# facebookresearch/wmar

Hardware: AMD Instinct MI355X
Metric: watermarked images/sec at 256x256 (16x16 tok), batch 64; detector p-value delta vs ref (higher is better)
Workload: dtype f32; 1 GPU; Taming cin_transformer (48L x 1536d x 24h, V=16384) + VQGAN f16/16384, 256x256, batch 64 per GPU, greenlist watermark delta=2 gamma=0.25 h=1 (linear/stratifiedrand), T=1 top-k 250 top-p 0.92; sample -> decode -> re-encode -> detect; random-init weights; batch_per_gpu=64, decode_loop=hipGraph replay, backend=nccl

## Files before the change

### include/wmar_hip.h

```cpp
#ifndef WMAR_HIP_H
#define WMAR_HIP_H

#include <stdint.h>

#ifdef __cplusplus
extern "C" {
#endif

#define WMAR_OK 0
#define WMAR_EINVAL (-1)
#define WMAR_EHIP (-2)
#define WMAR_ESHORT (-3)
#define WMAR_MAX_CONTEXT 16
#define WMAR_ENOMEM (-4)
#define WMAR_EMISSING (-5)
#define WMAR_ECALLBACK (-6)

#define WMAR_SEED_FIXED 0
#define WMAR_SEED_LINEAR 1
#define WMAR_SEED_SPATIAL 2
#define WMAR_SPLIT_RAND 0
#define WMAR_SPLIT_STRATIFIED 1

const char* wmar_last_error(void);
int wmar_version(void);

typedef struct wmar_key_params {
    uint64_t salt_key;
    const int64_t* alive_ids;
    int64_t n_alive;
    const int64_t* dead_ids;
    int64_t n_dead;
    int64_t vocab_size;
    double gamma;
    int32_t split_strategy;
    int32_t seed_strategy;
} wmar_key_params;

int64_t wmar_key_row_words(int64_t vocab_size);
int64_t wmar_key_table_rows(int32_t seed_strategy, int32_t context_size, int64_t max_token);
int wmar_key_table_build(const wmar_key_params* key, int64_t row0, int64_t n_rows, uint32_t* out_host,
                         int32_t n_threads);
int64_t wmar_key_greenlist(const wmar_key_params* key, uint64_t seed, int64_t* out_ids_host);

typedef struct wmar_wm_ctx {
    const uint32_t* table_dev;
    int64_t n_rows;
    int64_t vocab_size;
    int32_t seed_strategy;
    int32_t context_size;
    int32_t spatial_dim;
    float delta;
} wmar_wm_ctx;

int wmar_wm_process_logits(const wmar_wm_ctx* wm, float* logits_dev, int64_t B, const int64_t* past_ids_dev,
                           int64_t t, int64_t past_stride, void* stream);

int wmar_sample_fused(const wmar_wm_ctx* wm, const float* logits_dev, int64_t B, int64_t V,
                      const int64_t* past_ids_dev, int64_t t, int64_t past_stride, float temperature,
                      int32_t top_k, double top_p, const float* q_dev, float* scratch_dev,
                      int64_t* tok_out_dev, void* stream);

int wmar_detect(const wmar_wm_ctx* wm, double gamma, const int64_t* codes_dev, int64_t B, int64_t L,
                int32_t* n_scored_dev, int32_t* n_green_dev, double* pval_dev, int8_t* mask_dev,
                int64_t mask_stride, void* stream);
int64_t wmar_detect_num_ngrams(int32_t seed_strategy, int32_t context_size, int64_t L);

typedef struct wmar_gpt_config {
    int32_t vocab_size, block_size, n_layer, n_head, n_embd;
    int32_t max_batch;
} wmar_gpt_config;

typedef struct wmar_gpt wmar_gpt;

int wmar_gpt_create(const wmar_gpt_config* cfg, const char* const* names, const void* const* tensors_dev,
                    int32_t n_tensors, void* stream, wmar_gpt** out);
void wmar_gpt_destroy(wmar_gpt* g);
int64_t wmar_gpt_device_bytes(const wmar_gpt* g);

int wmar_gpt_decode_step(wmar_gpt* g, const int64_t* tok_dev, int64_t B, int32_t pos, float* logits_dev,
                         void* stream);

typedef struct wmar_sample_params {
    float temperature;
    int32_t top_k;
    double top_p;
    int32_t use_graph;
} wmar_sample_params;

int wmar_gpt_generate(wmar_gpt* g, const wmar_wm_ctx* wm, const wmar_sample_params* sp, const int64_t* cond_dev,
                      int64_t B, int32_t steps, const float* q_dev, int64_t* tokens_out_dev,
                      float* logits_trace_dev, void* stream);

typedef int (*wmar_logits_hook)(void* user, int32_t step, int64_t t);

int wmar_cfg_mix(const float* cond_dev, const float* img_dev, const float* uncond_dev, float* out_dev, int64_t B, int64_t V,
                 const float* scale_dev, const int32_t* step_dev, float g_text, float g_image, void* stream);

int wmar_gpt_generate_hooked(wmar_gpt* g, const wmar_sample_params* sp, const int64_t* cond_dev, int64_t B, int32_t steps,
                             const float* q_dev, int64_t* tokens_out_dev, float* logits_io_dev, int64_t* past_io_dev,
                             int64_t past_stride, wmar_logits_hook hook, void* user, void* stream);

#define WMAR_T_EMBED 0
#define WMAR_T_QKV 1
#define WMAR_T_ATTN 2
#define WMAR_T_PROJ 3
#define WMAR_T_RESID 4
#define WMAR_T_FC1 5
#define WMAR_T_FC2 6
#define WMAR_T_HEAD 7
#define WMAR_T_SAMPLE 8
#define WMAR_T_NCLASS 9
int wmar_gpt_check(wmar_gpt* g, void* stream);
int wmar_gpt_set_timing(wmar_gpt* g, int32_t enabled);
int wmar_gpt_set_attention_phases(wmar_gpt* g, int32_t one_wave_upto, int32_t two_waves_upto);
int wmar_gpt_profile_role(wmar_gpt* g, int32_t role, int64_t B, int32_t kv_len, int32_t iters, void* stream,
                          double* avg_us);
int wmar_gpt_plan_info(wmar_gpt* g, int64_t B, char* buf, int64_t buf_len);
int wmar_gpt_get_timing(wmar_gpt* g, double* total_us, int64_t* calls, double* step_ms);

typedef struct wmar_rar_config {
    int32_t hidden_size, num_hidden_layers, num_attention_heads, intermediate_size;
    int32_t image_seq_len, codebook_size, condition_num_classes;
    int32_t max_batch;
} wmar_rar_config;

typedef struct wmar_rar wmar_rar;

int wmar_rar_create(const wmar_rar_config* cfg, const char* const* names, const void* const* tensors_dev,
                    int32_t n_tensors, void* stream, wmar_rar** out);
void wmar_rar_destroy(wmar_rar* g);
int64_t wmar_rar_device_bytes(const wmar_rar* g);

int wmar_rar_forward_position(wmar_rar* g, const int64_t* tok_dev, const int64_t* cond_ids_dev, int64_t M, int32_t pos,
                              float* logits_dev, void* stream);

int wmar_rar_generate(wmar_rar* g, const wmar_wm_ctx* wm, const int64_t* class_ids_dev, int64_t B,
                      const float* cfg_scale_host, int32_t use_guidance, float temperature, const float* q_dev,
                      int64_t* tokens_out_dev, int32_t use_graph, void* stream);

int wmar_rar_generate_hooked(wmar_rar* g, const int64_t* class_ids_dev, int64_t B, const float* cfg_scale_host,
                             int32_t use_guidance, float temperature, const float* q_dev, int64_t* tokens_out_dev,
                             int32_t use_graph, float* logits_io_dev, int64_t* past_io_dev, int64_t past_stride,
                             wmar_logits_hook hook, void* user, void* stream);

// ... 159 lines not shown
```

### wmar_amd/_lib.py

```python
from __future__ import annotations

import ctypes as C
import os

HERE = os.path.dirname(os.path.abspath(__file__))
LIB_PATH = os.path.join(HERE, "libwmar_hip.so")

SYMBOLS = [
    "wmar_last_error", "wmar_version", "wmar_key_row_words", "wmar_key_table_rows", "wmar_key_table_build",
    "wmar_key_greenlist", "wmar_wm_process_logits", "wmar_sample_fused", "wmar_detect", "wmar_detect_num_ngrams",
    "wmar_gpt_create", "wmar_gpt_destroy", "wmar_gpt_device_bytes", "wmar_gpt_decode_step", "wmar_gpt_generate",
    "wmar_gpt_set_timing", "wmar_gpt_set_attention_phases", "wmar_gpt_get_timing", "wmar_gpt_profile_role", "wmar_gpt_plan_info", "wmar_gpt_check", "wmar_rar_create", "wmar_rar_destroy",
    "wmar_rar_device_bytes", "wmar_rar_forward_position", "wmar_rar_generate", "wmar_vq_create", "wmar_vq_destroy", "wmar_vq_device_bytes",
    "wmar_vq_decode", "wmar_vq_encode", "wmar_vq_probe_conv", "wmar_vq_probe_attn", "wmar_vq_probe_argmin", "wmar_mvq_create", "wmar_mvq_destroy", "wmar_mvq_device_bytes", "wmar_mvq_decode",
    "wmar_mvq_encode", "wmar_gumbel_key_build", "wmar_gumbel_sample", "wmar_gumbel_score", "wmar_gumbel_key_rows", "wmar_gumbel_score_ctx", "wmar_rar_generate_gumbel", "wmar_rar_generate_gumbel_ctx", "wmar_rar_check", "wmar_rar_launch_status",
    "wmar_cham_create", "wmar_cham_destroy", "wmar_cham_device_bytes", "wmar_cham_forward_tokens", "wmar_cham_generate_image",
    "wmar_cham_sample",
    "wmar_cfg_mix", "wmar_gpt_generate_hooked", "wmar_rar_generate_hooked", "wmar_cham_generate_image_hooked",
    "wmar_augment", "wmar_jpeg_workspace_bytes", "wmar_jpeg", "wmar_resample_coeffs", "wmar_image_ingest",
    "wmar_sync_positions", "wmar_sync_workspace_bytes", "wmar_sync_fit", "wmar_sync_rotate_labels",
    "wmar_comm_unique_id", "wmar_comm_init", "wmar_comm_bcast", "wmar_comm_allgather", "wmar_comm_rank", "wmar_comm_world", "wmar_comm_destroy",
]

WMAR_ESHORT = -3
WMAR_ECALLBACK = -6

LOGITS_HOOK = C.CFUNCTYPE(C.c_int, C.c_void_p, C.c_int32, C.c_int64)


class KeyParams(C.Structure):
    _fields_ = [("salt_key", C.c_uint64), ("alive_ids", C.POINTER(C.c_int64)), ("n_alive", C.c_int64),
                ("dead_ids", C.POINTER(C.c_int64)), ("n_dead", C.c_int64), ("vocab_size", C.c_int64),
                ("gamma", C.c_double), ("split_strategy", C.c_int32), ("seed_strategy", C.c_int32)]


class WmCtx(C.Structure):
    _fields_ = [("table_dev", C.c_void_p), ("n_rows", C.c_int64), ("vocab_size", C.c_int64),
                ("seed_strategy", C.c_int32), ("context_size", C.c_int32), ("spatial_dim", C.c_int32),
                ("delta", C.c_float)]


class GptConfig(C.Structure):
    _fields_ = [("vocab_size", C.c_int32), ("block_size", C.c_int32), ("n_layer", C.c_int32),
                ("n_head", C.c_int32), ("n_embd", C.c_int32), ("max_batch", C.c_int32)]


class RarConfig(C.Structure):
    _fields_ = [("hidden_size", C.c_int32), ("num_hidden_layers", C.c_int32), ("num_attention_heads", C.c_int32),
                ("intermediate_size", C.c_int32), ("image_seq_len", C.c_int32), ("codebook_size", C.c_int32),
                ("condition_num_classes", C.c_int32), ("max_batch", C.c_int32)]


class SampleParams(C.Structure):
    _fields_ = [("temperature", C.c_float), ("top_k", C.c_int32), ("top_p", C.c_double), ("use_graph", C.c_int32)]


class VqConfig(C.Structure):
    _fields_ = [("ch", C.c_int32), ("num_res_blocks", C.c_int32), ("resolution", C.c_int32),
                ("in_channels", C.c_int32), ("out_ch", C.c_int32), ("z_channels", C.c_int32),
                ("embed_dim", C.c_int32), ("n_embed", C.c_int32), ("n_levels", C.c_int32),
                ("ch_mult", C.c_int32 * 8), ("n_attn_res", C.c_int32), ("attn_resolutions", C.c_int32 * 8),
                ("max_batch", C.c_int32)]


class MvqConfig(C.Structure):
    _fields_ = [("hidden_channels", C.c_int32), ("num_res_blocks", C.c_int32), ("resolution", C.c_int32),
                ("num_channels", C.c_int32), ("z_channels", C.c_int32), ("num_embeddings", C.c_int32),
                ("n_levels", C.c_int32), ("channel_mult", C.c_int32 * 8), ("max_batch", C.c_int32)]


class ChamConfig(C.Structure):
    _fields_ = [("dim", C.c_int32), ("n_layers", C.c_int32), ("n_heads", C.c_int32), ("n_kv_heads", C.c_int32),
                ("vocab_size", C.c_int32), ("ffn_hidden", C.c_int32), ("norm_eps", C.c_float), ("rope_theta", C.c_float),
                ("qk_normalization", C.c_int32), ("swin_norm", C.c_int32), ("max_rows", C.c_int32),
                ("max_seq_len", C.c_int32), ("tensors_bf16", C.c_int32)]


class ChamSampleParams(C.Structure):
    _fields_ = [("temperature", C.c_float), ("top_p", C.c_double), ("guidance_scale_text", C.c_float),
                ("guidance_scale_image", C.c_float), ("use_graph", C.c_int32), ("pad_id", C.c_int32)]


class ImageDesc(C.Structure):
    _fields_ = [("offset", C.c_int64), ("width", C.c_int32), ("height", C.c_int32), ("channels", C.c_int32),
                ("new_width", C.c_int32), ("new_height", C.c_int32), ("crop_x0", C.c_int32), ("crop_y0", C.c_int32)]


class WmarError(RuntimeError):
    def __init__(self, code, msg):
        super().__init__(f"libwmar_hip: {msg} (status {code})")
        self.code = code


_LIB = None


def load():
    global _LIB
    if _LIB is not None:
        return _LIB
    import torch

    if not os.path.exists(LIB_PATH):
        raise ImportError(
            f"{LIB_PATH} is missing: build it with `python -m wmar_amd.build` (hipcc, gfx950). "
            "wmar_amd has no CPU fallback.")
    L = C.CDLL(LIB_PATH, mode=C.RTLD_GLOBAL)
    vp, i64, i32, f32, f64 = C.c_void_p, C.c_int64, C.c_int32, C.c_float, C.c_double
    L.wmar_last_error.restype = C.c_char_p
    L.wmar_key_row_words.restype = i64
    L.wmar_key_row_words.argtypes = [i64]
    L.wmar_key_table_rows.restype = i64
    L.wmar_key_table_rows.argtypes = [i32, i32, i64]
    L.wmar_key_table_build.argtypes = [C.POINTER(KeyParams), i64, i64, vp, i32]
    L.wmar_key_greenlist.restype = i64
    L.wmar_key_greenlist.argtypes = [C.POINTER(KeyParams), C.c_uint64, vp]
    L.wmar_wm_process_logits.argtypes = [C.POINTER(WmCtx), vp, i64, vp, i64, i64, vp]
    L.wmar_sample_fused.argtypes = [C.POINTER(WmCtx), vp, i64, i64, vp, i64, i64, f32, i32, f64, vp, vp, vp, vp]
    L.wmar_detect.argtypes = [C.POINTER(WmCtx), f64, vp, i64, i64, vp, vp, vp, vp, i64, vp]
    L.wmar_detect_num_ngrams.restype = i64
    L.wmar_detect_num_ngrams.argtypes = [i32, i32, i64]
    L.wmar_augment.argtypes = [i32, vp, vp, vp, i64, i32, i32, i32, i32, f64, f64, vp]
    L.wmar_jpeg_workspace_bytes.restype = i64
    L.wmar_jpeg_workspace_bytes.argtypes = [i64, i32, i32]
    L.wmar_jpeg.argtypes = [vp, vp, vp, i64, i64, i32, i32, i32, i32, i32, vp]
    L.wmar_resample_coeffs.argtypes = [i32, i32, i32, i32, vp, vp, vp, i32, C.POINTER(i32)]
    L.wmar_image_ingest.argtypes = [vp, i64, C.POINTER(ImageDesc), i64, i32, vp, vp, vp]
    L.wmar_sync_positions.argtypes = [vp, i64, i32, vp, vp, vp]
    L.wmar_sync_workspace_bytes.restype = i64
    L.wmar_sync_workspace_bytes.argtypes = [i64, i32]
    L.wmar_sync_fit.argtypes = [vp, i64, i32, vp, vp, vp, i64, vp]
    L.wmar_sync_rotate_labels.argtypes = [vp, i64, i32, i32, vp, vp, i64, vp]
    L.wmar_comm_unique_id.argtypes = [vp, i64]
    L.wmar_comm_init.argtypes = [vp, i64, i32, i32, C.POINTER(vp)]
    L.wmar_comm_bcast.argtypes = [vp, vp, i64, i32, vp]
    L.wmar_comm_allgather.argtypes = [vp, vp, vp, i64, vp]
    L.wmar_comm_rank.argtypes = [vp]
    L.wmar_comm_rank.restype = i32
    L.wmar_comm_world.argtypes = [vp]
    L.wmar_comm_world.restype = i32
    L.wmar_comm_destroy.argtypes = [vp]
    L.wmar_comm_destroy.restype = None
    L.wmar_gpt_create.argtypes = [C.POINTER(GptConfig), C.POINTER(C.c_char_p), C.POINTER(vp), i32, vp, C.POINTER(vp)]
    L.wmar_gpt_destroy.argtypes = [vp]
    L.wmar_gpt_destroy.restype = None
    L.wmar_gpt_device_bytes.restype = i64
    L.wmar_gpt_device_bytes.argtypes = [vp]
    L.wmar_gpt_decode_step.argtypes = [vp, vp, i64, i32, vp, vp]
    L.wmar_gpt_generate.argtypes = [vp, C.POINTER(WmCtx), C.POINTER(SampleParams), vp, i64, i32, vp, vp, vp, vp]
    L.wmar_gpt_set_timing.argtypes = [vp, i32]
    L.wmar_gpt_set_attention_phases.argtypes = [vp, i32, i32]
    L.wmar_gpt_profile_role.argtypes = [vp, i32, i64, i32, i32, vp, C.POINTER(f64)]
    L.wmar_gpt_get_timing.argtypes = [vp, C.POINTER(f64), C.POINTER(i64), C.POINTER(f64)]
    L.wmar_gpt_plan_info.argtypes = [vp, i64, C.c_char_p, i64]
    L.wmar_gpt_check.argtypes = [vp, vp]
    L.wmar_rar_create.argtypes = [C.POINTER(RarConfig), C.POINTER(C.c_char_p), C.POINTER(vp), i32, vp, C.POINTER(vp)]
    L.wmar_rar_destroy.argtypes = [vp]
    L.wmar_rar_destroy.restype = None
    L.wmar_rar_device_bytes.restype = i64
    L.wmar_rar_device_bytes.argtypes = [vp]
    L.wmar_rar_forward_position.argtypes = [vp, vp, vp, i64, i32, vp, vp]
    L.wmar_rar_generate.argtypes = [vp, C.POINTER(WmCtx), vp, i64, C.POINTER(f32), i32, f32, vp, vp, i32, vp]
    L.wmar_rar_generate_gumbel.argtypes = [vp, vp, i64, C.POINTER(f32), i32, f32, f32, i32, vp, vp, i32, vp]
    L.wmar_rar_generate_gumbel_ctx.argtypes = [vp, vp, i64, C.POINTER(f32), i32, f32, f32, i32, C.c_uint64, i32, vp, vp, i32, vp]
    L.wmar_rar_check.argtypes = [vp, vp]
    L.wmar_rar_launch_status.argtypes = [vp, C.POINTER(i32), C.POINTER(i32)]
    L.wmar_gumbel_key_build.argtypes = [C.c_uint64, i64, vp, vp, vp]
    L.wmar_gumbel_sample.argtypes = [vp, i64, i64, vp, i64, i32, f32, f32, i32, vp, vp]
    L.wmar_gumbel_score.argtypes = [vp, i64, i64, i64, vp, i64, vp, vp, vp]
    L.wmar_gumbel_key_rows.argtypes = [vp, i64, i64, vp, vp, vp, vp]
    L.wmar_gumbel_score_ctx.argtypes = [vp, i64, i64, i64, C.c_uint64, i32, vp, vp, vp, vp]
    if hasattr(L, "wmar_vq_create"):
        L.wmar_vq_create.argtypes = [C.POINTER(VqConfig), C.POINTER(C.c_char_p), C.POINTER(vp), i32, vp, C.POINTER(vp)]
        L.wmar_vq_destroy.argtypes = [vp]
        L.wmar_vq_destroy.restype = None
        L.wmar_vq_device_bytes.restype = i64
        L.wmar_vq_device_bytes.argtypes = [vp]
        L.wmar_vq_decode.argtypes = [vp, vp, i64, vp, vp]
        L.wmar_vq_encode.argtypes = [vp, vp, i64, vp, vp, vp]
        L.wmar_vq_probe_conv.argtypes = [vp, vp, i32, i32, i32, vp, vp, vp, vp, i32, i64, i32, i32, i32, i32, i32, vp, vp, C.c_char_p, i64, vp]
        L.wmar_vq_probe_attn.argtypes = [vp, vp, vp, i64, i32, i32, i32, vp, C.c_char_p, i64, vp]
        L.wmar_vq_probe_argmin.argtypes = [vp, i64, i32, vp, i32, vp, C.c_char_p, i64, vp]
    L.wmar_cham_create.argtypes = [C.POINTER(ChamConfig), C.POINTER(C.c_char_p), C.POINTER(vp), i32, vp, C.POINTER(vp)]
    L.wmar_cham_destroy.argtypes = [vp]
    L.wmar_cham_destroy.restype = None
    L.wmar_cham_device_bytes.restype = i64
    L.wmar_cham_device_bytes.argtypes = [vp]
    L.wmar_cham_forward_tokens.argtypes = [vp, vp, vp, i64, vp, vp]
    L.wmar_cham_generate_image.argtypes = [vp, C.POINTER(WmCtx), vp, vp, i64, C.POINTER(ChamSampleParams), vp, vp, i32, vp, i32, vp, vp]
    L.wmar_cham_sample.argtypes = [C.POINTER(WmCtx), vp, i64, i64, vp, i64, i64, f32, f64, f32, f32, vp, vp, i32, vp, vp, vp, vp]
    L.wmar_cfg_mix.argtypes = [vp, vp, vp, vp, i64, i64, vp, vp, f32, f32, vp]
    L.wmar_gpt_generate_hooked.argtypes = [vp, C.POINTER(SampleParams), vp, i64, i32, vp, vp, vp, vp, i64, LOGITS_HOOK, vp, vp]
    L.wmar_rar_generate_hooked.argtypes = [vp, vp, i64, C.POINTER(f32), i32, f32, vp, vp, i32, vp, vp, i64, LOGITS_HOOK, vp, vp]
    L.wmar_cham_generate_image_hooked.argtypes = [vp, vp, vp, i64, C.POINTER(ChamSampleParams), vp, vp, i32, vp, i32, vp, vp, vp, i64,
                                                  LOGITS_HOOK, vp, vp]
    L.wmar_mvq_create.argtypes = [C.POINTER(MvqConfig), C.POINTER(C.c_char_p), C.POINTER(vp), i32, vp, C.POINTER(vp)]
    L.wmar_mvq_destroy.argtypes = [vp]
    L.wmar_mvq_destroy.restype = None
    L.wmar_mvq_device_bytes.restype = i64
    L.wmar_mvq_device_bytes.argtypes = [vp]
    L.wmar_mvq_decode.argtypes = [vp, vp, i64, vp, vp]
    L.wmar_mvq_encode.argtypes = [vp, vp, i64, vp, vp, vp]
    _LIB = L
# ... 23 lines not shown
```

### wmar_amd/csrc/decoder_kernels.h

```cpp
#pragma once
#include <cstdint>

#include "sampler.h"
#include "bx_split.h"

namespace wmar {

using f32x16 = __attribute__((ext_vector_type(16))) float;
using f32x4 = __attribute__((ext_vector_type(4))) float;

__device__ __forceinline__ float4 ld_nt(const float4* p) {
    f32x4 v = __builtin_nontemporal_load((const f32x4*)p);
    return make_float4(v.x, v.y, v.z, v.w);
}

__device__ __forceinline__ void st_out(float4* p, const float4 v) {
#ifndef WMAR_PLAIN_STORES
    const f32x4 q = {v.x, v.y, v.z, v.w};
    asm volatile("global_store_dwordx4 %0, %1, off sc1\n\ts_nop 1" :: "v"(p), "v"(q) : "memory");
#else
    *p = v;
#endif
}
using f32x2 = __attribute__((ext_vector_type(2))) float;
// ... 649 lines not shown
        mu = (float)mean;
        rstd = rsqrtf((float)var_f64(sq * invK, mean) + 1e-5f);
    }
    for (int gi = w; gi < 6; gi += 4) {
        float o[4] = {0.f, 0.f, 0.f, 0.f};
#pragma unroll
        for (int ww = 0; ww < 4; ++ww) {
            const float4 t = red[ww][gi][lane];
            o[0] += t.x; o[1] += t.y; o[2] += t.z; o[3] += t.w;
        }
        const int m = gi < 4 ? 16 * gi + (lane & 15) : lane;
        const int n = tile * 24 + (gi < 4 ? 4 * (lane >> 4) : 16 + 4 * (gi - 4));
        const float mm = __shfl(mu, m), rs = __shfl(rstd, m);
        const float4 cc = gi < 4 ? ccA_ : ccB_;
        const float4 bb = gi < 4 ? bbA_ : bbB_;
        o[0] = gelu_erf(rs * (o[0] - mm * cc.x) + bb.x); o[1] = gelu_erf(rs * (o[1] - mm * cc.y) + bb.y);
        o[2] = gelu_erf(rs * (o[2] - mm * cc.z) + bb.z); o[3] = gelu_erf(rs * (o[3] - mm * cc.w) + bb.w);
        st_out(a.out + ((long long)(n >> 3) * 2 + (m >> 5)) * 64 + (m & 31) + 32 * ((n >> 2) & 1), make_float4(o[0], o[1], o[2], o[3]));
    }
    WMAR_ST_END(a.trace, blockIdx.x)
#ifdef WMAR_FX_TRACE
    if (a.trace && threadIdx.x == 0) {
        asm volatile("s_waitcnt vmcnt(0)" ::: "memory");
        unsigned long long* t = a.trace + (long long)blockIdx.x * 4;
        t[0] = tr0; t[1] = tr1; t[2] = tr2; t[3] = __builtin_amdgcn_s_memtime();
    }
#endif
}

constexpr int QX_CK = 4;
#ifndef QX_ABL
#define QX_ABL 0
#endif
#define WMAR_QX_SYNC() if (!(QX_ABL & 2)) __syncthreads();
#ifndef QX_SPLIT
#define QX_SPLIT 2
#endif

struct QkvxArgs {
    const float4* Wp;
    const float4* x_in;
    float4* x_out;
    const float4* slabs;
    long long slab_stride;
    int n_hi;
    const float* bias;
    double* stats;
    float4* out;
    long long out_stride;
    int KB, NT, S, cap;
    int nkeep;
    unsigned long long* trace;
    unsigned long long* trace_chunks;
};

template <int MTW, int S_IN>
__global__ __launch_bounds__(512) void k_qkvx(QkvxArgs a) {
    __shared__ __attribute__((aligned(16))) float4 xs[2][QX_CK][MTW][64];
    __shared__ double red[4][MTW][64][2];
    const int lane = threadIdx.x & 63;
    const int w = __builtin_amdgcn_readfirstlane(threadIdx.x >> 6);
    const int half = lane >> 5;
    const int G = a.NT >> 2;
    const int j = (int)(blockIdx.x & 7) * a.cap + (int)(blockIdx.x >> 3);
    if (j >= G * a.S) return;
    const int s = j / G, g = j - s * G;
    const int kb0 = (int)((unsigned)s * (unsigned)a.KB / (unsigned)a.S);
    const int kb1 = (int)((unsigned)(s + 1) * (unsigned)a.KB / (unsigned)a.S);
    const int nkb = kb1 - kb0, nch = (nkb + QX_CK - 1) / QX_CK;
    const bool keeper = g == 0;

    if (w >= 4) {
        const int sw = w - 4;
        double sum[MTW], sq[MTW];
#pragma unroll
        for (int i = 0; i < MTW; ++i) { sum[i] = 0.0; sq[i] = 0.0; }
        float4 xvA[MTW], bbA, slA[S_IN > 0 ? S_IN : 1][MTW];
        float4 xvB[MTW], bbB, slB[S_IN > 0 ? S_IN : 1][MTW];
        int skbA = 0, skbB = 0;
#define WMAR_QX_ISSUE(XV, BB, SL, SKB, C)                                                              \
    {                                                                                                   \
        SKB = kb0 + (C) * QX_CK + sw;                                                                   \
        const int kk = SKB < kb1 ? SKB : kb1 - 1;                                                       \
        const long long idx = (long long)kk * MTW * 64 + lane;                                          \
        _Pragma("unroll") for (int i = 0; i < MTW; ++i) XV[i] = a.x_in[idx + i * 64];                   \
        if (S_IN > 0) {                                                                                 \
            BB = *(const float4*)(a.bias + kk * 8 + 4 * half);                                          \
            _Pragma("unroll") for (int si = 0; si < S_IN; ++si)                                         \
                _Pragma("unroll") for (int i = 0; i < MTW; ++i)                                         \
                    SL[si][i] = a.slabs[(long long)si * a.slab_stride + idx + i * 64];                  \
        }                                                                                               \
    }
#define WMAR_QX_FINISH(XV, BB, SL, SKB, BUF)                                                           \
    if (SKB < kb1) {                                                                                    \
        const bool short_tile = a.n_hi > 0 && (SKB >> 2) >= a.n_hi;                                     \
        _Pragma("unroll") for (int i = 0; i < MTW; ++i) {                                               \
            float4 r = XV[i];                                                                           \
            if (S_IN > 0) {                                                                             \
                float4 t = SL[0][i];                                                                    \
                _Pragma("unroll") for (int si = 1; si < S_IN; ++si)                                     \
                    if (!(si == S_IN - 1 && short_tile)) {                                              \
                        t.x += SL[si][i].x; t.y += SL[si][i].y; t.z += SL[si][i].z; t.w += SL[si][i].w; \
                    }                                                                                   \
                r = make_float4(r.x + (BB.x + t.x), r.y + (BB.y + t.y), r.z + (BB.z + t.z), r.w + (BB.w + t.w)); \
            }                                                                                           \
            xs[BUF][sw][i][lane] = r;                                                                   \
// ... 129 lines not shown
#endif
#pragma unroll
    for (int i = 0; i < MTW; ++i)
#pragma unroll
        for (int q4 = 0; q4 < 4; ++q4)
            st_out(a.out + (long long)s * a.out_stride + ((long long)(nt * 4 + q4) * MTW + i) * 64 + lane,
                   make_float4(acc[i][q4 * 4 + 0], acc[i][q4 * 4 + 1], acc[i][q4 * 4 + 2], acc[i][q4 * 4 + 3]));
    if (keeper) __syncthreads();
#ifdef WMAR_QX_TRACE
    if (a.trace && lane == 0) {
        asm volatile("s_waitcnt vmcnt(0)" ::: "memory");
        unsigned long long* t = a.trace + ((long long)j * 4 + w) * 4;
        t[0] = tr0; t[1] = tr1; t[2] = tr2; t[3] = __builtin_amdgcn_s_memtime();
        if (a.trace_chunks) for (int i = 0; i < 8; ++i) a.trace_chunks[((long long)j * 4 + w) * 8 + i] = trc[i] ? trc[i] - tr1 : 0;
    }
#endif
}

template <int MTW>
static int launch_qkvx_mt(const QkvxArgs& q, int S_in, hipStream_t st) {
    const dim3 grid((unsigned)(8 * q.cap));
    switch (S_in) {
#define WMAR_QX_CASE(N) case N: hipLaunchKernelGGL((k_qkvx<MTW, N>), grid, dim3(512), 0, st, q); break;
        WMAR_QX_CASE(0) WMAR_QX_CASE(1) WMAR_QX_CASE(2) WMAR_QX_CASE(3) WMAR_QX_CASE(4)
        WMAR_QX_CASE(5) WMAR_QX_CASE(6) WMAR_QX_CASE(7) WMAR_QX_CASE(8)
#undef WMAR_QX_CASE
        default: set_error("qkvx: bad slab count %d", S_in); return WMAR_EINVAL;
    }
    return launch_status("k_qkvx");
}
static int launch_qkvx(const QkvxArgs& q, int MT, int S_in, hipStream_t st) {
    if (MT == 1) return launch_qkvx_mt<1>(q, S_in, st);
    if (MT == 2) return launch_qkvx_mt<2>(q, S_in, st);
    set_error("qkvx: %d row tiles unsupported", MT);
    return WMAR_EINVAL;
}

static __global__ void k_pack_bx(const float* __restrict__ W, const float* __restrict__ gamma, float4* __restrict__ Wq, int N, int K,
                                      int tile_off) {
    const long long idx = (long long)blockIdx.x * blockDim.x + threadIdx.x;
    const int KU = K / 16;
    if (idx >= (long long)(N / 32) * KU * 128) return;
    const int lane = (int)(idx & 63), hf = (int)((idx >> 6) & 1);
    const long long r = idx >> 7;
    const int ku = (int)(r % KU), tile = (int)(r / KU);
    const int k = ku * 16 + 8 * (lane >> 5) + 4 * hf;
    const float* p = W + (long long)(tile * 32 + (lane & 31)) * K + k;
    float4 v = make_float4(p[0], p[1], p[2], p[3]);
    if (gamma) { v.x *= gamma[k]; v.y *= gamma[k + 1]; v.z *= gamma[k + 2]; v.w *= gamma[k + 3]; }
    Wq[idx + (long long)tile_off * KU * 128] = v;
}

constexpr int QX_TR_STRIDE = 36;
template <int S_IN>
__global__ __launch_bounds__(512) void k_qkvx_bx(QkvxArgs a) {
    constexpr int MTW = 2;
    __shared__ __attribute__((aligned(16))) u32x4 xq[2][2][MTW][3][64];
    __shared__ __attribute__((aligned(16))) float tr_s[4][32 * QX_TR_STRIDE];
    __shared__ double red[4][MTW][64][2];
    const int lane = threadIdx.x & 63;
    const int w = __builtin_amdgcn_readfirstlane(threadIdx.x >> 6);
    const int half = lane >> 5;
    const int G = a.NT >> 2;
    const int j = (int)(blockIdx.x & 7) * a.cap + (int)(blockIdx.x >> 3);
    if (j >= G * a.S) return;
    const int s = j / G, g = j - s * G;
    const int KU = a.KB >> 1;
    const int kb0 = 2 * (int)((unsigned)s * (unsigned)KU / (unsigned)a.S);
    const int kb1 = 2 * (int)((unsigned)(s + 1) * (unsigned)KU / (unsigned)a.S);
    const int nkb = kb1 - kb0, nch = (nkb + QX_CK - 1) / QX_CK;
    const bool keeper = g < a.nkeep;

    if (w >= 4) {
        const int sw = w - 4;
        double sum[MTW], sq[MTW];
#pragma unroll
        for (int i = 0; i < MTW; ++i) { sum[i] = 0.0; sq[i] = 0.0; }
        float4 xvA[MTW], bbA, slA[S_IN > 0 ? S_IN : 1][MTW];
        float4 xvB[MTW], bbB, slB[S_IN > 0 ? S_IN : 1][MTW];
        int skbA = 0, skbB = 0;
#define WMAR_QX_ISSUE(XV, BB, SL, SKB, C)                                                              \
    {                                                                                                   \
        SKB = kb0 + (C) * QX_CK + sw;                                                                   \
        const int kk = SKB < kb1 ? SKB : kb1 - 1;                                                       \
        const long long idx = (long long)kk * MTW * 64 + lane;                                          \
        _Pragma("unroll") for (int i = 0; i < MTW; ++i) XV[i] = a.x_in[idx + i * 64];                   \
        if (S_IN > 0) {                                                                                 \
            BB = *(const float4*)(a.bias + kk * 8 + 4 * half);                                          \
            _Pragma("unroll") for (int si = 0; si < S_IN; ++si)                                         \
                _Pragma("unroll") for (int i = 0; i < MTW; ++i)                                         \
                    SL[si][i] = a.slabs[(long long)si * a.slab_stride + idx + i * 64];                  \
        }                                                                                               \
    }
#define WMAR_QX_FINISH(XV, BB, SL, SKB, BUF, CIDX)                                                     \
    if (SKB < kb1) {                                                                                    \
        const bool short_tile = a.n_hi > 0 && (SKB >> 2) >= a.n_hi;                                     \
        _Pragma("unroll") for (int i = 0; i < MTW; ++i) {                                               \
            float4 r = XV[i];                                                                           \
            if (S_IN > 0) {                                                                             \
                float4 t = SL[0][i];                                                                    \
                _Pragma("unroll") for (int si = 1; si < S_IN; ++si)                                     \
                    if (!(si == S_IN - 1 && short_tile)) {                                              \
                        t.x += SL[si][i].x; t.y += SL[si][i].y; t.z += SL[si][i].z; t.w += SL[si][i].w; \
                    }                                                                                   \
                r = make_float4(r.x + (BB.x + t.x), r.y + (BB.y + t.y), r.z + (BB.z + t.z), r.w + (BB.w + t.w)); \
            }                                                                                           \
            unsigned h0, m0, l0, h1, m1, l1;                                                            \
            bx_split2(r.x, r.y, h0, m0, l0);                                                            \
            bx_split2(r.z, r.w, h1, m1, l1);                                                            \
            u32x2* d = (u32x2*)&xq[BUF][sw >> 1][i][0][(lane & 31) + 32 * (sw & 1)] + half;             \
            d[0] = u32x2{h0, h1}; d[128] = u32x2{m0, m1}; d[256] = u32x2{l0, l1};                       \
            if (keeper && (CIDX) % a.nkeep == g) {                                                      \
                a.x_out[((long long)SKB * MTW + i) * 64 + lane] = r;                                    \
                sum[i] += (double)r.x + (double)r.y + (double)r.z + (double)r.w;                        \
                sq[i] += sq4_f64(r);                        \
            }                                                                                           \
        }                                                                                               \
    }
        WMAR_QX_ISSUE(xvA, bbA, slA, skbA, 0)
        WMAR_QX_ISSUE(xvB, bbB, slB, skbB, 1)
        __builtin_amdgcn_sched_barrier(0);
        WMAR_QX_FINISH(xvA, bbA, slA, skbA, 0, 0)
        __builtin_amdgcn_sched_barrier(0);
        WMAR_QX_ISSUE(xvA, bbA, slA, skbA, 2)
        __builtin_amdgcn_sched_barrier(0);
        __syncthreads();
        for (int c = 0; c + 1 < nch; c += 2) {
            WMAR_QX_FINISH(xvB, bbB, slB, skbB, 1, c + 1)
            __builtin_amdgcn_sched_barrier(0);
            WMAR_QX_ISSUE(xvB, bbB, slB, skbB, c + 3)
            __builtin_amdgcn_sched_barrier(0);
            __syncthreads();
            if (c + 2 >= nch) break;
            WMAR_QX_FINISH(xvA, bbA, slA, skbA, 0, c + 2)
            __builtin_amdgcn_sched_barrier(0);
            WMAR_QX_ISSUE(xvA, bbA, slA, skbA, c + 4)
            __builtin_amdgcn_sched_barrier(0);
            __syncthreads();
        }
#undef WMAR_QX_ISSUE
#undef WMAR_QX_FINISH
        if (keeper) {
#pragma unroll
            for (int i = 0; i < MTW; ++i) {
                red[sw][i][lane][0] = sum[i]; red[sw][i][lane][1] = sq[i];
            }
            __syncthreads();
            const int t = threadIdx.x - 256;
            if (t < 32 * MTW) {
                const int i = t >> 5, r = t & 31;
                double ts = 0, tss = 0;
// ... 49 lines not shown
    __builtin_amdgcn_sched_barrier(0);                                                                  \
    if ((C) + 1 < nch) {                                                                                \
        __syncthreads();                                                                                \
        WMAR_QX_READ(XNEXT, BUFNEXT)                                                                    \
    }                                                                                                   \
    __builtin_amdgcn_sched_barrier(0);                                                                  \
    WMAR_QX_MMA(WCUR, XCUR, C, 1)                                                                       \
    __builtin_amdgcn_sched_barrier(0);

    WMAR_QX_W(w0, 0)
    WMAR_QX_W(w1, 1)
    WMAR_QX_W(w2, 2)
    __syncthreads();
    WMAR_ST_LANDED(2)
    WMAR_QX_READ(xfA, 0)
    for (int c = 0; c < nch; c += 4) {
        WMAR_QX_STEP(c, w0, w3, xfA, xfB, 1)
        if (c + 1 >= nch) break;
        WMAR_QX_STEP(c + 1, w1, w0, xfB, xfA, 0)
        if (c + 2 >= nch) break;
        WMAR_QX_STEP(c + 2, w2, w1, xfA, xfB, 1)
        if (c + 3 >= nch) break;
        WMAR_QX_STEP(c + 3, w3, w2, xfB, xfA, 0)
    }
    WMAR_ST(3)
#undef WMAR_QX_W
#undef WMAR_QX_READ
#undef WMAR_QX_MMA
#undef WMAR_QX_MFMA
#undef WMAR_QX_BF
#undef WMAR_QX_STEP
#pragma unroll
    for (int i = 0; i < MTW; ++i) {
        float* T = &tr_s[w][0];
#pragma unroll
        for (int q4 = 0; q4 < 4; ++q4)
            *(float4*)(T + (lane & 31) * QX_TR_STRIDE + 8 * q4 + 4 * half) =
                make_float4(acc[i][q4 * 4 + 0], acc[i][q4 * 4 + 1], acc[i][q4 * 4 + 2], acc[i][q4 * 4 + 3]);
        __builtin_amdgcn_wave_barrier();
        asm volatile("s_waitcnt lgkmcnt(0)" ::: "memory");
#pragma unroll
        for (int it = 0; it < 4; ++it) {
            const int row = (lane >> 3) + 8 * it, cg = lane & 7;
            const float4 v = *(const float4*)(T + row * QX_TR_STRIDE + 4 * cg);
            st_out(a.out + (long long)s * a.out_stride + ((long long)(32 * i + row) * (a.NT * 32) + nt * 32 + 4 * cg) / 4, v);
        }
        __builtin_amdgcn_wave_barrier();
        asm volatile("s_waitcnt lgkmcnt(0)" ::: "memory");
    }
    WMAR_ST_END(a.trace, j)
    if (keeper) __syncthreads();
}

static int launch_qkvx_bx(const QkvxArgs& q, int S_in, hipStream_t st) {
    const dim3 grid((unsigned)(8 * q.cap));
    switch (S_in) {
#define WMAR_QX_CASE(N) case N: hipLaunchKernelGGL((k_qkvx_bx<N>), grid, dim3(512), 0, st, q); break;
        WMAR_QX_CASE(0) WMAR_QX_CASE(1) WMAR_QX_CASE(2) WMAR_QX_CASE(3) WMAR_QX_CASE(4)
        WMAR_QX_CASE(5) WMAR_QX_CASE(6) WMAR_QX_CASE(7) WMAR_QX_CASE(8)
#undef WMAR_QX_CASE
        default: set_error("qkvx_bx: bad slab count %d", S_in); return WMAR_EINVAL;
    }
    return launch_status("k_qkvx_bx");
}


struct BxArgs {
    const float4* Wq;
    const u32x4* Xq;
    float4* out;
    long long slab_stride;
    int KU;
    int S;
    const float* bias;
    u32x4* outq;
    int rowmajor;
    int N;
};

#define WMAR_BX_MFMA(A, B, C) C = __builtin_amdgcn_mfma_f32_32x32x16_bf16(A, B, C, 0, 0, 0)

template <int NT, int PER, int MTW = 2, bool GELU = false, int NW = 4, bool XF = false>
__global__ __launch_bounds__(NW * 64) void k_bx(BxArgs a) {
    constexpr int XR = XF ? 2 * MTW : 3 * MTW;
    constexpr int ROWS = NT * 4 * MTW;
    __shared__ __attribute__((aligned(16))) float4 red[NW][ROWS][64];
    const int lane = threadIdx.x & 63;
    const int w = __builtin_amdgcn_readfirstlane(threadIdx.x >> 6);
    const int grp = (int)blockIdx.x / a.S, ks = (int)blockIdx.x % a.S;
    const int u0 = (ks * NW + w) * PER;
    f32x16 acc[NT][MTW];
#pragma unroll
    for (int t = 0; t < NT; ++t)
#pragma unroll
        for (int i = 0; i < MTW; ++i)
#pragma unroll
            for (int r = 0; r < 16; ++r) acc[t][i][r] = 0.f;
    const float4* wp = a.Wq + ((long long)grp * NT * a.KU + u0) * 128 + lane;
    const long long wt = (long long)a.KU * 128;
    const u32x4* xp = XF ? a.Xq + ((long long)(2 * u0 + (lane >> 5)) * MTW) * 64 + (lane & 31)
                         : a.Xq + (long long)u0 * XR * 64 + lane;
    float4 wr[NT][2];
    u32x4 xr[XR], xr2[XF ? XR : 1];
#define WMAR_BX_LOADW(U)                                                                           \
    { _Pragma("unroll") for (int t = 0; t < NT; ++t) {                                             \
        wr[t][0] = ld_nt(wp + t * wt + (long long)(U) * 128);                                      \
        wr[t][1] = ld_nt(wp + t * wt + (long long)(U) * 128 + 64); } }
#define WMAR_BX_LOADXF(XB, U)                                                                      \
// ... 809 lines not shown
```

### wmar_amd/csrc/gpt.hip

```cpp
#include <cstdint>
#include <map>
#include <string>
#include <vector>

#include "decoder_host.h"
#include "decode_small.h"
#include "decode_persist.h"


using namespace wmar;

struct LayerW {
    float4 *wqkv, *wproj, *wfc1, *wfc2;
    float4* wfc1x16 = nullptr;
    float2* wfc1x8 = nullptr;
    float4* wqkvx_bx = nullptr;
    float4* wproj_bx = nullptr;
    float *bqkv, *bproj, *bfc1, *bfc2, *cqkv, *cfc1;
};

struct SmallW {
    float *wqkv = nullptr, *bqkv = nullptr, *wproj = nullptr, *bproj = nullptr, *wfc1 = nullptr, *bfc1 = nullptr, *wfc2 = nullptr, *bfc2 = nullptr;
    float *ln1w = nullptr, *ln1b = nullptr, *ln2w = nullptr, *ln2b = nullptr;
};

struct wmar_gpt {
    wmar_gpt_config cfg{};
    int D = 0, H = 0, hd = 0, V = 0, L = 0, Tmax = 0, Bmax = 0, MTmax = 0;
    DeviceArena mem;
    std::vector<LayerW> layers;
    std::vector<SmallW> sw;
    float *whead_rm = nullptr, *lnfw = nullptr, *lnfb = nullptr;
    float *xs = nullptr, *ys = nullptr, *hs = nullptr, *qs = nullptr;
    bool small_ok = false;
    float* sw_arena = nullptr;
    unsigned* ss_bar = nullptr;
    bool persist_ok = false;
    bool ps_enqueued = false;
    bool xr_enqueued = false;
    float *tok_emb = nullptr, *pos_emb = nullptr, *bhead = nullptr, *chead = nullptr;
    float4* whead = nullptr;
    float4 *x = nullptr, *x2 = nullptr, *y = nullptr, *hbuf = nullptr, *slabs = nullptr, *qkv_slabs = nullptr;
    u32x4* yq = nullptr;
    float* qbuf = nullptr;
    double* stats = nullptr;
    double* stats_q = nullptr;
    float *kcache = nullptr, *vcache = nullptr;
    float *logits = nullptr, *scratch = nullptr;
    long long* past = nullptr;
    int *pos_dev = nullptr, *step_dev = nullptr;
    hipEvent_t ev0 = nullptr;
    static constexpr int N_PHASE = 3;
    GraphSlots<N_PHASE> gr;
    GraphSlots<N_PHASE + 1> grh;
    unsigned long long hook_key[12] = {0};
    int att_nw = 2;
    unsigned long long graph_key[12] = {0};
    int att_t1 = 1 << 30, att_t2 = 1 << 30;
    bool att_user = false;
    int att_phase(int kv, int64_t B) const {
        if (!att_user && B * H < 512) return kv <= 128 ? 1 : 2;
        return kv <= att_t1 ? 0 : (kv <= att_t2 ? 1 : 2);
    }
    static int phase_waves(int ph) { return ph == 0 ? 1 : (ph == 1 ? 2 : 4); }
    int timing = 0;
    bool no_bx_qkv = false, no_bx_proj = false;
    unsigned* xsync = nullptr;
    bool xcd_ok = false;
    bool no_xr = false;
    int inject_fail = 0;
    int fallbacks = 0;
    unsigned long long* dbg_sums = nullptr; int dbg_slot = 0;
    unsigned long long* stamps = nullptr;
    unsigned long long* stamp_slot(int l, int role) const {
        return stamps ? stamps + ((long long)(l * 5 + role) * WMAR_STAMP_UNITS) * 8 : nullptr;
    }
    bool no_bx = false;
    int force_s[3] = {0, 0, 0};
    double step_ms = 0.0;
    struct Span { int cls; hipEvent_t a, b; };
    std::vector<Span> spans;
    std::vector<hipEvent_t> ev_pool;
    size_t ev_used = 0;
    bool span_on = false;
    double cls_us[WMAR_T_NCLASS] = {0};
    int64_t cls_calls[WMAR_T_NCLASS] = {0};
    hipEvent_t next_event() {
        if (ev_used == ev_pool.size()) {
            hipEvent_t e = nullptr;
            (void)hipEventCreate(&e);
            ev_pool.push_back(e);
        }
        return ev_pool[ev_used++];
    }
    void span_begin(int cls, hipStream_t st) {
        if (!span_on) return;
        Span s{cls, next_event(), next_event()};
        (void)hipEventRecord(s.a, st);
        spans.push_back(s);
    }
    void span_end(hipStream_t st) {
// ... 45 lines not shown
    ResidArgs r{};
    int S_qkv = 1, S_proj = 1, S_fc2 = 1;
    int fc2_hi = 0;
    int S_qx = 0;
    float4* xcur = nullptr;
    bool proj_bx = false;
    bool proj_xr = false;
    int nch_ln2 = 0;
    bool small = false;
    bool persist = false;

    StepPlan(wmar_gpt* g_, int64_t B_, const StepIO& io_, hipStream_t st_) : g(g_), B(B_), io(io_), st(st_) {
        small = B <= SG_MAX_ROWS && g->small_ok;
        persist = small && B <= SS_MAX_ROWS && g->persist_ok;
        MT = mt_for(B); D = g->D; KBD = D / 8; KBF = 4 * D / 8; nch = stat_chunks(KBD);
        act = (long long)KBD * MT * 64;
        r.x = g->x; r.stats = g->stats; r.KB = KBD; r.MT = MT; r.n_chunks = nch;
        r.tok_emb = g->tok_emb; r.pos_emb = g->pos_emb; r.tok = io.tok; r.tok_stride = io.tok_stride;
        r.tok_use_pos = io.tok_use_pos; r.pos_dev = g->pos_dev; r.B = (int)B; r.K = D;
        r.slabs = g->slabs; r.slab_stride = act;
        xcur = g->x;
        S_qkv = g->force_s[0] > 0 ? (g->force_s[0] > QKV_SLABS_MAX ? QKV_SLABS_MAX : g->force_s[0]) : 1;
        S_proj = g->force_s[1] > 0 ? g->force_s[1] : split_for(D / 32, KBD);
        S_fc2 = g->force_s[2] > 0 ? g->force_s[2] : ((MT % 2 == 0 && KBF >= 128) ? 4 : split_for(D / 32, KBF));
        if (g->force_s[2] <= 0 && MT == 2 && KBF >= 256) {
            const int NTd = D / 32;
            const int Slo = 256 / NTd;
            if (Slo >= 2 && Slo < MAX_SLABS && NTd * Slo <= 256) { S_fc2 = Slo; fc2_hi = 256 - NTd * Slo; if (fc2_hi >= NTd) fc2_hi = 0; }
        }
        const int NTq = 3 * D / 32;
        if (g->force_s[0] <= 0 && NTq % 4 == 0 && MT <= 2 && S_fc2 + (fc2_hi > 0 ? 1 : 0) <= MAX_SLABS) {
            const int G = NTq / 4;
            int S = 256 / G;
            if (S > QKV_SLABS_MAX) S = QKV_SLABS_MAX;
            if (S > KBD / QX_CK) S = KBD / QX_CK;
            if (S >= 1) S_qx = S;
        }
        proj_bx = MT == 2 && g->yq && g->layers[0].wproj_bx && !g->no_bx && !g->no_bx_proj && g->force_s[1] <= 0;
        if (proj_bx) S_proj = D / BX_KSLICE;
        proj_xr = proj_bx && g->xcd_ok && !g->no_xr && S_proj == 4 && (D / 32) % 8 == 0 && (D / 32 / 8) * S_proj <= 32 && (D / 32 / 8) % 2 == 0;
        nch_ln2 = proj_xr ? 16 : nch;
    }
    void dbg(const void* p, long long bytes) {
#ifdef WMAR_DEV_KNOBS
        if (!g->dbg_sums || g->dbg_slot >= 4096) return;
        hipLaunchKernelGGL(k_dbg_sum, dim3(512), dim3(256), 0, st, (const uint32_t*)p, bytes / 4, g->dbg_sums + g->dbg_slot++);
#else
        (void)p; (void)bytes;
#endif
    }
    bool qkv_bx() const { return S_qx > 0 && MT == 2 && g->layers[0].wqkvx_bx && !g->no_bx && !g->no_bx_qkv; }
    bool fc1_x() const { return MT == 2 && g->layers[0].wfc1x16 && nch_ln2 <= 16; }
    int qx_nkeep() const { const int G = 3 * D / 128; return G >= 4 && S_qx * 4 <= STAT_CHUNKS_MAX ? 4 : 1; }
    static bool head_narrow() { static int v = -1; if (v < 0) v = getenv("WMAR_HEAD_NARROW") ? 1 : 0; return v != 0; }
    int split_for(int NT, int KB) const { return pick_split(MT % 2 == 0 ? NT * (MT / 2) : NT * MT, KB, 4); }
    GemmArgs base() const {
        GemmArgs a{};
        a.MT = MT; a.B = (int)B; a.stats = g->stats; a.n_chunks = nch; a.K = D;
        a.pos_dev = g->pos_dev; a.D = D; a.H = g->H; a.hd = g->hd; a.Tmax = g->Tmax;
        return a;
    }
    SgArgs sg_base() const {
        SgArgs a{};
        a.pos_dev = g->pos_dev; a.D = D; a.H = g->H; a.Tmax = g->Tmax;
        return a;
    }
    int embed() {
        if (small) {
            SeArgs e{g->tok_emb, g->pos_emb, g->xs, io.tok, io.tok_stride, io.tok_use_pos, g->pos_dev, D};
            g->span_begin(WMAR_T_EMBED, st);
            hipLaunchKernelGGL(k_sembed, dim3((unsigned)((D / 4 + 255) / 256), (unsigned)B), dim3(256), 0, st, e);
            g->span_end(st);
            return launch_status("k_sembed");
        }
        r.x = xcur;
        g->span_begin(WMAR_T_EMBED, st);
        hipLaunchKernelGGL((k_resid_stats<true, 0>), dim3(nch * MT), dim3(256), 0, st, r);
        g->span_end(st);
        return launch_status("k_resid_stats<embed>");
    }
    int resid(const float* bias, int S, int n_hi = 0) {
        r.x = xcur;
        r.S = S + (n_hi > 0 ? 1 : 0); r.bias = bias; r.n_hi = n_hi;
        g->span_begin(WMAR_T_RESID, st);
        int rc = launch_resid(r, nch * MT, st);
        g->span_end(st);
        return rc;
    }
    int qkvx(int l, const float* prev_bias) {
        QkvxArgs q{};
        const LayerW& w = g->layers[l];
        float4* xout = (xcur == g->x) ? g->x2 : g->x;
        q.Wp = w.wqkv; q.x_in = xcur; q.x_out = xout;
        q.slabs = g->slabs; q.slab_stride = act;
        const int S_in = prev_bias ? S_fc2 + (fc2_hi > 0 ? 1 : 0) : 0;
        q.n_hi = prev_bias ? fc2_hi : 0; q.bias = prev_bias;
        q.stats = g->stats_q; q.out = g->qkv_slabs; q.out_stride = 3 * act;
        q.KB = KBD; q.NT = 3 * D / 32; q.S = S_qx;
        q.cap = ((q.NT / 4) * q.S + 7) / 8;
        q.nkeep = qx_nkeep();
        q.trace = g->stamp_slot(l, 0);
        g->span_begin(WMAR_T_QKV, st);
        int rc;
        if (qkv_bx()) { q.Wp = w.wqkvx_bx; rc = launch_qkvx_bx(q, S_in, st); }
        else rc = launch_qkvx(q, MT, S_in, st);
        g->span_end(st);
        xcur = xout;
        return rc;
    }
    int qkv_small(int l) {
        const SmallW& w = g->sw[l];
        const long long lstride = (long long)g->Bmax * g->H * g->Tmax * g->hd;
        SgArgs a = sg_base();
        a.W = w.wqkv; a.bias = g->layers[l].bqkv; a.c1 = g->layers[l].cqkv; a.x = g->xs; a.gamma = w.ln1w; a.out = g->qs;
        a.kcache = g->kcache + l * lstride; a.vcache = g->vcache + l * lstride; a.N = 3 * D; a.K = D;
        g->span_begin(WMAR_T_QKV, st);
        const int rc = launch_sgemv<3, 3, SG_QKV>(a, (int)B, st);
        g->span_end(st);
        return rc;
    }
    int qkv(int l) {
        GemmArgs a = base();
        const LayerW& w = g->layers[l];
        a.Wp = w.wqkv; a.Xp = xcur; a.KB = KBD; a.NT = 3 * D / 32;
        a.out_packed = g->qkv_slabs; a.slab_stride = 3 * act;
        int S = 1;
        g->span_begin(WMAR_T_QKV, st);
        int rc = gemm_split(a, &S, st, S_qkv);
        g->span_end(st);
        return rc;
    }
    int attn(int l) {
        const LayerW& w = g->layers[l];
        const long long lstride = (long long)g->Bmax * g->H * g->Tmax * g->hd;
        if (small) {
            SaArgs s{g->qs, g->kcache + l * lstride, g->vcache + l * lstride, g->ys, g->pos_dev, g->H, g->Tmax, D, 1.0f / sqrtf((float)g->hd)};
            g->span_begin(WMAR_T_ATTN, st);
            hipLaunchKernelGGL(k_sattn, dim3((unsigned)(B * g->H)), dim3(256), 0, st, s);
            g->span_end(st);
            return launch_status("k_sattn");
        }
        AttnArgs t{};
        t.qkv_slabs = g->qkv_slabs; t.slab_stride = 3 * act; t.K = D; t.invK = 1.0 / (double)D;
        if (S_qx > 0) { t.S = S_qx; t.stats = g->stats_q; t.n_chunks = qkv_bx() ? S_qx * qx_nkeep() : S_qx; }
        else { t.S = S_qkv; t.stats = g->stats; t.n_chunks = nch; }
        t.c1 = w.cqkv; t.bias = w.bqkv;
        t.rowmajor = qkv_bx() ? 1 : 0;
        t.kcache = g->kcache + l * lstride; t.vcache = g->vcache + l * lstride; t.y = g->y; t.yq = proj_bx ? g->yq : nullptr; t.pos_dev = g->pos_dev;
        t.D = D; t.H = g->H; t.Tmax = g->Tmax; t.MT = MT; t.scale = 1.0f / sqrtf((float)g->hd);
        t.trace = g->stamp_slot(l, 1);
        int nwa = g->att_nw;
#ifdef WMAR_DEV_KNOBS
        { const char* e = getenv("WMAR_ATT_DBG"); t.dbg = e ? atoi(e) : 0; }
        { const char* e = getenv("WMAR_ATT_NW"); if (e) nwa = atoi(e); }
#endif
        const dim3 grid((unsigned)(B * g->H));
        g->span_begin(WMAR_T_ATTN, st);
// ... 111 lines not shown
            a.W = g->whead_rm; a.bias = g->bhead; a.c1 = g->chead; a.x = g->xs; a.gamma = g->lnfw; a.out = io.logits; a.N = g->V; a.K = D;
            g->span_begin(WMAR_T_HEAD, st);
            const int rc = launch_sgemv<4, 8, SG_HEAD>(a, (int)B, st);
            g->span_end(st);
            return rc;
        }
        GemmArgs h = base();
        h.Wp = g->whead; h.Xp = xcur; h.KB = KBD; h.NT = g->V / 32;
        h.bias = g->bhead; h.c1 = g->chead; h.logits = io.logits; h.V = g->V;
        g->span_begin(WMAR_T_HEAD, st);
        int rc = WMAR_OK;
        if (MT == 2 && h.NT % 2 == 0 && h.NT / 2 <= 512 && !head_narrow()) {
            h.S = 1;
            rc = launch_gemm<2, 4, EPI_LOGITS, true, 0, GEMM_STAGE, true, 2>(h, st);
        } else {
        const int MG = (MT % 2 == 0) ? MT / 2 : MT;
        const int per = 256 / MG > 0 ? 256 / MG : 1;
        const int NTall = h.NT;
        for (int nt0 = 0; nt0 < NTall && rc == WMAR_OK; nt0 += per) {
            GemmArgs p = h;
            p.NT = NTall - nt0 < per ? NTall - nt0 : per;
            p.Wp = h.Wp + (long long)nt0 * h.KB * 64;
            p.bias = h.bias ? h.bias + (long long)nt0 * 32 : nullptr;
            p.c1 = h.c1 + (long long)nt0 * 32;
            p.logits = h.logits + (long long)nt0 * 32;
            rc = gemm_dispatch<EPI_LOGITS, true>(p, false, st);
        }
        }
        g->span_end(st);
        return rc;
    }
};

int enqueue_step(wmar_gpt* g, int64_t B, const StepIO& io, hipStream_t st) {
    StepPlan p(g, B, io, st);
    int rc;
    const long long actb = p.act * 16, Mpad = p.MT * 32;
#ifdef WMAR_DEV_KNOBS
    if (g->dbg_sums) { g->dbg_slot = 0; if (hipMemsetAsync(g->dbg_sums, 0, 4096 * 8, st) != hipSuccess) return WMAR_EHIP; }
#endif
    if (p.persist) {
        SsArgs a{};
        a.arena = g->sw_arena; a.L = g->L; a.tok_emb = g->tok_emb; a.pos_emb = g->pos_emb; a.whead = g->whead_rm; a.lnfw = g->lnfw; a.lnfb = g->lnfb;
        a.tok = io.tok; a.tok_stride = io.tok_stride; a.tok_use_pos = io.tok_use_pos;
        a.xs = g->xs; a.ys = g->ys; a.hs = g->hs; a.qs = g->qs; a.kcache = g->kcache; a.vcache = g->vcache;
        a.lstride = (long long)g->Bmax * g->H * g->Tmax * g->hd; a.logits = io.logits; a.V = g->V; a.pos_dev = g->pos_dev;
        a.D = g->D; a.H = g->H; a.Tmax = g->Tmax; a.bar = g->ss_bar;
        g->span_begin(WMAR_T_QKV, st);
        rc = launch_sstep(a, (int)B, st);
        g->span_end(st);
        g->ps_enqueued = true;
        return rc;
    }
    if ((rc = p.embed())) return rc;
    if (p.small) {
        for (int l = 0; l < g->L; ++l) {
            if ((rc = p.qkv_small(l))) return rc;
            if ((rc = p.attn(l))) return rc;
            if ((rc = p.proj(l))) return rc;
            if ((rc = p.fc1(l))) return rc;
            if ((rc = p.fc2(l))) return rc;
        }
        return p.head();
    }
    p.dbg(p.xcur, actb); p.dbg(g->stats, p.nch * Mpad * 16);
    for (int l = 0; l < g->L; ++l) {
        if (p.S_qx > 0) {
            if ((rc = p.qkvx(l, l > 0 ? g->layers[l - 1].bfc2 : nullptr))) return rc;
            p.dbg(p.xcur, actb); p.dbg(g->stats_q, p.S_qx * Mpad * 16); p.dbg(g->qkv_slabs, p.S_qx * 3 * actb);
        } else {
            if (l > 0 && (rc = p.resid(g->layers[l - 1].bfc2, p.S_fc2, p.fc2_hi))) return rc;
            if ((rc = p.qkv(l))) return rc;
            p.dbg(p.xcur, actb); p.dbg(g->stats, p.nch * Mpad * 16); p.dbg(g->qkv_slabs, 3 * actb);
        }
        if ((rc = p.attn(l))) return rc;
        if (p.proj_bx) p.dbg(g->yq, (long long)p.D / 16 * 2 * 3 * 64 * 16); else p.dbg(g->y, actb);
        {
            const long long lstride = (long long)g->Bmax * g->H * g->Tmax * g->hd;
            p.dbg(g->kcache + l * lstride, lstride * 4); p.dbg(g->vcache + l * lstride, lstride * 4);
        }
        if ((rc = p.proj(l))) return rc;
        p.dbg(g->slabs, p.S_proj * actb);
        if (!p.proj_xr && (rc = p.resid(g->layers[l].bproj, p.S_proj))) return rc;
        p.dbg(p.xcur, actb); p.dbg(g->stats, p.nch_ln2 * Mpad * 16);
        if ((rc = p.fc1(l))) return rc;
        p.dbg(g->hbuf, 4 * actb);
        if ((rc = p.fc2(l))) return rc;
        p.dbg(g->slabs, p.S_fc2 * actb);
    }
    if ((rc = p.resid(g->layers[g->L - 1].bfc2, p.S_fc2, p.fc2_hi))) return rc;
    p.dbg(p.xcur, actb); p.dbg(g->stats, p.nch * Mpad * 16);
    return p.head();
}

}

extern "C" {

int wmar_gpt_create(const wmar_gpt_config* cfg, const char* const* names, const void* const* tensors_dev,
                    int32_t n_tensors, void* stream, wmar_gpt** out) {
    WMAR_REQUIRE(cfg && names && tensors_dev && out, "gpt_create: null argument");
    WMAR_REQUIRE(cfg->n_embd % cfg->n_head == 0, "n_embd %% n_head != 0");
    const int D = cfg->n_embd, H = cfg->n_head, hd = D / H, V = cfg->vocab_size, L = cfg->n_layer;
    WMAR_REQUIRE(D % 32 == 0 && V % 32 == 0 && D <= 8192, "n_embd (<= 8192) and vocab_size must be multiples of 32 (got %d, %d)", D, V);
    WMAR_REQUIRE(hd == 32 || hd == 64 || hd == 128, "head_dim %d unsupported (32, 64, 128)", hd);
    WMAR_REQUIRE(cfg->max_batch >= 1 && cfg->max_batch <= 128, "max_batch must be in 1..128");
    WMAR_REQUIRE(cfg->block_size >= 1 && L >= 1, "bad block_size / n_layer");
// ... 95 lines not shown
    if (rc == WMAR_OK && D == 2 * SG_SEG && hd == 64 && !getenv("WMAR_NO_SMALL")) {
        g->sw.resize(L);
        const size_t DD = (size_t)D * D;
        WMAR_TRY(g->mem.alloc(&g->sw_arena, (size_t)L * SS_LAYER_FLOATS));
        for (int l = 0; l < L && rc == WMAR_OK; ++l) {
            std::string p = "blocks." + std::to_string(l) + ".";
            SmallW& w = g->sw[l];
            float* base = g->sw_arena + (size_t)l * SS_LAYER_FLOATS;
            w.wqkv = base + SS_OFF_WQKV; w.wproj = base + SS_OFF_WPROJ; w.wfc1 = base + SS_OFF_WFC1; w.wfc2 = base + SS_OFF_WFC2;
            w.bqkv = base + SS_OFF_BQKV; w.bproj = base + SS_OFF_BPROJ; w.bfc1 = base + SS_OFF_BFC1; w.bfc2 = base + SS_OFF_BFC2;
            w.ln1w = base + SS_OFF_LN1W; w.ln1b = base + SS_OFF_LN1B; w.ln2w = base + SS_OFF_LN2W; w.ln2b = base + SS_OFF_LN2B;
            hipError_t e = hipSuccess;
            auto cp = [&](float* dst, const std::string& key, size_t n) {
                if (e == hipSuccess) e = hipMemcpyAsync(dst, tm.get(p + key), n * 4, hipMemcpyDeviceToDevice, st);
            };
            cp(w.wqkv, "attn.query.weight", DD); cp(w.wqkv + DD, "attn.key.weight", DD); cp(w.wqkv + 2 * DD, "attn.value.weight", DD);
            cp(w.bqkv, "attn.query.bias", D); cp(w.bqkv + D, "attn.key.bias", D); cp(w.bqkv + 2 * D, "attn.value.bias", D);
            cp(w.wproj, "attn.proj.weight", DD); cp(w.bproj, "attn.proj.bias", D);
            cp(w.wfc1, "mlp.0.weight", 4 * DD); cp(w.bfc1, "mlp.0.bias", (size_t)4 * D);
            cp(w.wfc2, "mlp.2.weight", 4 * DD); cp(w.bfc2, "mlp.2.bias", D);
            cp(w.ln1w, "ln1.weight", D); cp(w.ln1b, "ln1.bias", D); cp(w.ln2w, "ln2.weight", D); cp(w.ln2b, "ln2.bias", D);
            if (e != hipSuccess) { set_error("gpt_create: %s", hipGetErrorString(e)); rc = WMAR_EHIP; }
        }
        WMAR_TRY(copy_vec(g, &g->whead_rm, hw, (size_t)V * D, st));
        WMAR_TRY(copy_vec(g, &g->lnfw, lfw, D, st));
        WMAR_TRY(copy_vec(g, &g->lnfb, lfb, D, st));
        WMAR_TRY(g->mem.alloc(&g->xs, (size_t)SG_MAX_ROWS * D));
        WMAR_TRY(g->mem.alloc(&g->ys, (size_t)SG_MAX_ROWS * D));
        WMAR_TRY(g->mem.alloc(&g->hs, (size_t)SG_MAX_ROWS * 4 * D));
        WMAR_TRY(g->mem.alloc(&g->qs, (size_t)SG_MAX_ROWS * D));
        g->small_ok = rc == WMAR_OK;
        static_assert(SSD == 2 * SG_SEG, "arena offsets are for n_embd 1536");
        if (g->small_ok && getenv("WMAR_PERSIST") && !getenv("WMAR_NO_PERSIST")) {
            WMAR_TRY(g->mem.alloc_zero(&g->ss_bar, (size_t)SS_BAR_WORDS, st));
            if (rc == WMAR_OK) g->persist_ok = grid_resident(sstep_blocks_per_cu(), SS_WGS) && xcd_grouping_ok(SS_WGS, SS_THREADS, st);
        }
    }
    const size_t Mpad = (size_t)g->MTmax * 32;
    WMAR_TRY(g->mem.alloc_zero(&g->x, Mpad * D / 4, st));
    WMAR_TRY(g->mem.alloc_zero(&g->x2, Mpad * D / 4, st));
    WMAR_TRY(g->mem.alloc_zero(&g->y, Mpad * D / 4, st));
    WMAR_TRY(g->mem.alloc_zero(&g->hbuf, Mpad * 4 * D / 4, st));
    WMAR_TRY(g->mem.alloc(&g->slabs, (size_t)MAX_SLABS * Mpad * D / 4));
    WMAR_TRY(g->mem.alloc(&g->qkv_slabs, (size_t)MAX_SLABS * Mpad * 3 * D / 4));
    if (g->MTmax >= 2 && D % BX_KSLICE == 0) WMAR_TRY(g->mem.alloc_zero(&g->yq, (size_t)D / 16 * 2 * 3 * 64, st));
    WMAR_TRY(g->mem.alloc_zero(&g->qbuf, Mpad * D, st));
    WMAR_TRY(g->mem.alloc(&g->stats, (size_t)STAT_CHUNKS_MAX * Mpad * 2));
    WMAR_TRY(g->mem.alloc(&g->stats_q, (size_t)QKV_SLABS_MAX * 4 * Mpad * 2));
    const size_t kv = (size_t)L * g->Bmax * H * g->Tmax * hd;
    WMAR_TRY(g->mem.alloc_zero(&g->kcache, kv, st));
    WMAR_TRY(g->mem.alloc_zero(&g->vcache, kv, st));
    WMAR_TRY(g->mem.alloc(&g->logits, (size_t)g->Bmax * V));
    WMAR_TRY(g->mem.alloc(&g->scratch, (size_t)g->Bmax * V));
    WMAR_TRY(g->mem.alloc_zero(&g->past, (size_t)g->Bmax * (g->Tmax + 1), st));
    WMAR_TRY(g->mem.alloc(&g->pos_dev, 4));
    WMAR_TRY(g->mem.alloc_zero(&g->xsync, 8 * 64 + 64, st));
    g->step_dev = g->pos_dev + 1;
    WMAR_TRY(g->gr.init());
    WMAR_TRY(g->grh.init());
    if (rc == WMAR_OK) {
        hipError_t e = hipEventCreate(&g->ev0);
        if (e == hipSuccess) e = hipStreamSynchronize(st);
        if (e != hipSuccess) { set_error("gpt_create: %s", hipGetErrorString(e)); rc = WMAR_EHIP; }
    }
    if (rc == WMAR_OK && g->MTmax >= 2 && g->yq) {
        g->no_xr = getenv("WMAR_NO_XR") != nullptr;
        const bool xr4 = getenv("WMAR_XR_NW4") != nullptr;
        const long long blocks = (long long)(D / 32) * 4;
        g->xcd_ok = xcd_grouping_ok(192, 256, st) &&
                    (xr4 ? grid_resident(k_bx_xr<BX_PER, 4>, 256, blocks) : grid_resident(k_bx_xr<BX_PER / 2, 4, 8>, 512, blocks));
        { const char* e = getenv("WMAR_INJECT_SYNC_FAIL"); g->inject_fail = (e && atoi(e) > 0) ? 1 : 0; }
    }
    if (rc != WMAR_OK) { delete g; return rc; }
    *out = g;
    return WMAR_OK;
}

static int gpt_persist_failed(wmar_gpt* g, hipStream_t st) {
    if (!g->ss_bar || !g->persist_ok || !g->ps_enqueued) return 0;
    g->ps_enqueued = false;
    unsigned f = 0;
    WMAR_HIP_CHECK(hipMemcpyAsync(&f, g->ss_bar + 8 * 64 + 64, 4, hipMemcpyDeviceToHost, st));
    WMAR_HIP_CHECK(hipStreamSynchronize(st));
    if (!f) return 0;
    g->gr.drop();
    g->grh.drop();
    WMAR_HIP_CHECK(hipMemsetAsync(g->ss_bar, 0, SS_BAR_WORDS * 4, st));
    g->persist_ok = false;
    g->fallbacks += 1;
    fprintf(stderr, "wmar_amd: the persistent decode step (k_sstep) gave up waiting at its device-wide barrier; this engine continues on the "
                    "five-launch small-batch plan (the call is re-run; wmar_gpt_plan_info reports barrier_fallbacks)\n");
    return 1;
}
static int gpt_sync_failed(wmar_gpt* g, hipStream_t st) {
    if (const int pf = gpt_persist_failed(g, st)) return pf;
    if (!g->xsync || !g->xcd_ok || g->no_xr || !g->xr_enqueued) return 0;
    g->xr_enqueued = false;
    unsigned f[2] = {0, 0};
    WMAR_HIP_CHECK(hipMemcpyAsync(f, g->xsync + 8 * 64, 8, hipMemcpyDeviceToHost, st));
    WMAR_HIP_CHECK(hipStreamSynchronize(st));
    if (!f[0] && !f[1]) return 0;
    g->gr.drop();
    g->grh.drop();
    WMAR_HIP_CHECK(hipMemsetAsync(g->xsync, 0, (8 * 64 + 64) * 4, st));
    g->xcd_ok = false;
    g->fallbacks += 1;
// ... 53 lines not shown
    auto one = [&](int it) -> int {
        const int l = it % ncycle;
        switch (role) {
            case WMAR_T_EMBED: return p.embed();
            case WMAR_T_QKV: if (p.small) return p.qkv_small(l); p.xcur = g->x; return p.S_qx > 0 ? p.qkvx(l, g->layers[l].bfc2) : p.qkv(l);
            case WMAR_T_ATTN: return p.attn(l);
            case WMAR_T_PROJ: return p.proj(l);
            case WMAR_T_RESID: if (p.small) { set_error("profile_role: the small-batch path has no residual launch"); return WMAR_EINVAL; } return p.resid(g->layers[l].bproj, p.S_proj);
            case WMAR_T_FC1: return p.fc1(l);
            case WMAR_T_FC2: return p.fc2(l);
            case WMAR_T_HEAD: return p.head();
            default: set_error("profile_role: unknown role %d", role); return WMAR_EINVAL;
        }
    };
    const bool was = g->span_on;
    g->span_on = false;
    int rc = WMAR_OK;
    for (int i = 0; i < 3 && rc == WMAR_OK; ++i) rc = one(i);
    if (rc == WMAR_OK && hipEventRecord(g->ev0, st) != hipSuccess) rc = WMAR_EHIP;
    for (int i = 0; i < iters && rc == WMAR_OK; ++i) rc = one(i + 3);
    if (rc == WMAR_OK && hipEventRecord(g->gr.done, st) != hipSuccess) rc = WMAR_EHIP;
    g->span_on = was;
    if (rc) return rc;
    WMAR_HIP_CHECK(hipEventSynchronize(g->gr.done));
    float ms = 0.f;
    WMAR_HIP_CHECK(hipEventElapsedTime(&ms, g->ev0, g->gr.done));
    *avg_us = (double)ms * 1000.0 / iters;
    return WMAR_OK;
}

int wmar_gpt_plan_info(wmar_gpt* g, int64_t B, char* buf, int64_t buf_len) {
    WMAR_REQUIRE(g && buf && buf_len > 0, "plan_info: null argument");
    WMAR_REQUIRE(B >= 1 && B <= g->Bmax, "plan_info: batch outside 1..%d", g->Bmax);
    StepIO io{g->past, (long long)g->Tmax + 1, 0, g->logits};
    StepPlan p(g, B, io, nullptr);
    if (p.persist) {
        const int n = snprintf(buf, (size_t)buf_len,
                               "qkv=k_sstep phase (the arithmetic of k_sgemv<QKV>, weights streamed across the barriers);attn=k_sstep phase;proj=k_sstep phase;resid=none;"
                               "resid_launches_per_step=0;fc1=k_sstep phase;fc2=k_sstep phase;head=k_sstep phase;barrier_fallbacks=%d;"
                               "path=persistent step: one launch, %d device-wide barriers (decode_persist.h)", g->fallbacks, 5 * g->L + 1);
        WMAR_REQUIRE(n > 0 && n < buf_len, "plan_info: buffer of %lld bytes too small", (long long)buf_len);
        return WMAR_OK;
    }
    if (p.small) {
        const int n = snprintf(buf, (size_t)buf_len,
                               "qkv=k_sgemv<QKV> (row-major weight stream, LN1 + bias + cache append inside, %d columns per workgroup);"
                               "attn=k_sattn (4 waves per (sequence, head));proj=k_sgemv<PROJ> (residual added in place);resid=none;"
                               "resid_launches_per_step=0;fc1=k_sgemv<FC1> (LN2 + bias + GELU inside);fc2=k_sgemv<FC2> (8 K segments, residual added in place);"
                               "head=k_sgemv<HEAD> (ln_f inside);barrier_fallbacks=%d;path=small-batch streaming (decode_small.h)",
                               sg_cols_wg<3, 3, SG_QKV>(), g->fallbacks);
        WMAR_REQUIRE(n > 0 && n < buf_len, "plan_info: buffer of %lld bytes too small", (long long)buf_len);
        return WMAR_OK;
    }
    char qkv[96], proj[160], fc1[96], fc2[96];
    const int S_in = p.S_fc2 + (p.fc2_hi > 0 ? 1 : 0);
    if (p.qkv_bx()) snprintf(qkv, sizeof qkv, "k_qkvx_bx<%d> (bf16 pipe, %d K slices)", S_in, p.S_qx);
    else if (p.S_qx > 0) snprintf(qkv, sizeof qkv, "k_qkvx<%d,%d> (fp32 MFMA, %d K slices)", p.MT, S_in, p.S_qx);
    else snprintf(qkv, sizeof qkv, "k_gemm<EPI_PACKED> (fp32 MFMA, %d K slices) after k_resid_stats", p.S_qkv);
    if (p.proj_xr) snprintf(proj, sizeof proj, "k_bx_xr<%d,4> (bf16 pipe, 4 K slices + XCD-local reduction: residual fold and LN2 statistics inside)", BX_PER);
    else if (p.proj_bx) snprintf(proj, sizeof proj, "k_bx<1,%d> (bf16 pipe, %d K slices)", BX_PER, p.S_proj);
    else snprintf(proj, sizeof proj, "k_gemm<EPI_PACKED> (fp32 MFMA, %d K slices)", p.S_proj);
    if (p.fc1_x()) snprintf(fc1, sizeof fc1, "k_fc1x (fp32 MFMA, 24-column tiles, whole K)");
    else snprintf(fc1, sizeof fc1, "k_gemm<EPI_GELU,LN> (fp32 MFMA, whole K)");
    snprintf(fc2, sizeof fc2, "k_gemm<EPI_PACKED> (fp32 MFMA, %d%s K slices)", p.S_fc2, p.fc2_hi > 0 ? "/+1" : "");
    char attn[96];
    const int w0 = wmar_gpt::phase_waves(g->att_phase(1, B)), w1 = wmar_gpt::phase_waves(g->att_phase(g->Tmax / 2, B)),
              w2 = wmar_gpt::phase_waves(g->att_phase(g->Tmax, B));
    if (w0 == w1 && w1 == w2) snprintf(attn, sizeof attn, "k_attn_decode<%d,%d>", g->hd, w1);
    else snprintf(attn, sizeof attn, "k_attn_decode<%d,%d> (%d / %d / %d waves at 1 / %d / %d cached rows)", g->hd, w1, w0, w1, w2, g->Tmax / 2, g->Tmax);
    const int n = snprintf(buf, (size_t)buf_len, "qkv=%s;attn=%s;proj=%s;resid=k_resid_stats;resid_launches_per_step=%d;fc1=%s;fc2=%s;head=k_gemm<EPI_LOGITS,LN> (fp32 MFMA);barrier_fallbacks=%d",
                           qkv, attn, proj, p.proj_xr ? 1 : g->L + 1, fc1, fc2, g->fallbacks);
    WMAR_REQUIRE(n > 0 && n < buf_len, "plan_info: buffer of %lld bytes too small", (long long)buf_len);
    return WMAR_OK;
}

#ifdef WMAR_STAMPS
int wmar_gpt_debug_stamps(wmar_gpt* g, unsigned long long* out, long long n_u64) {
    WMAR_REQUIRE(g && g->stamps && out, "debug_stamps: not enabled (WMAR_STAMPS=1 at creation of a -DWMAR_STAMPS build)");
    const long long n = (long long)g->L * 5 * WMAR_STAMP_UNITS * 8;
    WMAR_HIP_CHECK(hipDeviceSynchronize());
    WMAR_HIP_CHECK(hipMemcpy(out, g->stamps, (size_t)(n_u64 < n ? n_u64 : n) * 8, hipMemcpyDeviceToHost));
    return WMAR_OK;
}
#endif

#ifdef WMAR_DEV_KNOBS
int wmar_gpt_debug_sums(wmar_gpt* g, unsigned long long* out, int n_out, int* n_used) {
    WMAR_REQUIRE(g && g->dbg_sums && out, "debug_sums: not enabled (WMAR_DBG_SUMS=1 at creation)");
    WMAR_HIP_CHECK(hipDeviceSynchronize());
    WMAR_HIP_CHECK(hipMemcpy(out, g->dbg_sums, (size_t)(n_out < 4096 ? n_out : 4096) * 8, hipMemcpyDeviceToHost));
    if (n_used) *n_used = g->dbg_slot;
    return WMAR_OK;
}
#endif

#ifdef WMAR_DEV_KNOBS
int wmar_gpt_debug_small(wmar_gpt* g, int which, float* out) {
    WMAR_REQUIRE(g && g->small_ok && out && which >= 0 && which <= 3, "debug_small: bad argument");
    WMAR_HIP_CHECK(hipDeviceSynchronize());
    const float* src = which == 0 ? g->xs : which == 1 ? g->qs : which == 2 ? g->ys : g->hs;
    WMAR_HIP_CHECK(hipMemcpy(out, src, (size_t)SG_MAX_ROWS * (which == 3 ? 4 : 1) * g->D * 4, hipMemcpyDeviceToHost));
    return WMAR_OK;
}
#endif

#ifdef WMAR_DEV_KNOBS
int wmar_gpt_debug_kv_row(wmar_gpt* g, int which, int pos, float* out) {
    WMAR_REQUIRE(g && out && pos >= 0 && pos < g->Tmax, "debug_kv_row: bad argument");
    WMAR_HIP_CHECK(hipDeviceSynchronize());
    const float* src = (which ? g->vcache : g->kcache) + (long long)pos * g->hd;
    WMAR_HIP_CHECK(hipMemcpy2D(out, (size_t)g->hd * 4, src, (size_t)g->Tmax * g->hd * 4, (size_t)g->hd * 4,
                               (size_t)g->L * g->Bmax * g->H, hipMemcpyDeviceToHost));
    return WMAR_OK;
}
#endif


int wmar_gpt_set_attention_phases(wmar_gpt* g, int32_t one_wave_upto, int32_t two_waves_upto) {
    WMAR_REQUIRE(g, "set_attention_phases: null argument");
    if (one_wave_upto < 0 && two_waves_upto < 0) {
        if (g->att_user) g->gr.drop();
        g->att_t1 = 1 << 30; g->att_t2 = 1 << 30; g->att_user = false;
        return WMAR_OK;
    }
    WMAR_REQUIRE(one_wave_upto >= 0 && two_waves_upto >= one_wave_upto, "set_attention_phases: bad thresholds");
    if (!g->att_user || g->att_t1 != one_wave_upto || g->att_t2 != two_waves_upto) g->gr.drop();
    g->att_t1 = one_wave_upto; g->att_t2 = two_waves_upto; g->att_user = true;
    return WMAR_OK;
}

int wmar_gpt_set_timing(wmar_gpt* g, int32_t enabled) { if (!g) return WMAR_EINVAL; g->timing = enabled; return WMAR_OK; }
int wmar_gpt_get_timing(wmar_gpt* g, double* total_us, int64_t* calls, double* step_ms) {
    if (!g) return WMAR_EINVAL;
    for (int i = 0; i < WMAR_T_NCLASS; ++i) {
        if (total_us) total_us[i] = g->cls_us[i];
        if (calls) calls[i] = g->cls_calls[i];
    }
    if (step_ms) *step_ms = g->step_ms;
    return WMAR_OK;
}

#ifndef WMAR_GRAPH_STEPS_DEFAULT
#define WMAR_GRAPH_STEPS_DEFAULT 4
#endif
static int gpt_generate_once(wmar_gpt* g, const wmar_wm_ctx* wm, const wmar_sample_params* sp, const int64_t* cond_dev,
                             int64_t B, int32_t steps, const float* q_dev, int64_t* tokens_out_dev,
                             float* logits_trace_dev, void* stream) {
    WMAR_REQUIRE(g && sp && cond_dev && q_dev && tokens_out_dev, "generate: null argument");
    WMAR_REQUIRE(B >= 1 && B <= g->Bmax, "generate: batch %lld outside 1..%d", (long long)B, g->Bmax);
    WMAR_REQUIRE(steps >= 1 && steps <= g->Tmax, "generate: steps %d outside 1..block_size %d", steps, g->Tmax);
    WMAR_REQUIRE(!(sp->top_p >= 0) || sp->top_p <= 1.0, "`top_p` has to be a float > 0 and < 1, but is %f", sp->top_p);
    if (wm) {
        WMAR_REQUIRE(wm->table_dev && wm->vocab_size == g->V, "generate: watermark vocab mismatch");
        WMAR_REQUIRE(wm->context_size >= 0 && wm->context_size <= WMAR_MAX_CONTEXT, "context size unsupported");
        WMAR_REQUIRE(wm->seed_strategy != WMAR_SEED_SPATIAL || wm->context_size == 1 || wm->context_size == 3,
                     "Spatial seeding only implemented for context size in [1,3]");
    }
    hipStream_t st = (hipStream_t)stream;
    const long long pstride = g->Tmax + 1;
    if (int rc = gpt_inject(g, st)) return rc;
    WMAR_HIP_CHECK(hipMemcpy2DAsync(g->past, pstride * 8, cond_dev, 8, 8, (size_t)B, hipMemcpyDeviceToDevice, st));
    WMAR_HIP_CHECK(hipMemsetAsync(g->pos_dev, 0, 8, st));

    SampArgs a{};
    a.wm = make_wm(wm);
    a.logits = g->logits; a.V = g->V; a.past = g->past; a.past_stride = pstride;
    a.t_dev = g->step_dev;
    a.temperature = sp->temperature; a.top_k = sp->top_k; a.use_top_p = sp->top_p >= 0;
    a.top_p_thr = (float)(1.0 - sp->top_p);
    a.q = q_dev; a.q_step_stride = (long long)B * g->V; a.step_dev = g->step_dev;
    a.scratch = a.V > 65536 ? g->scratch : nullptr;
    a.tok_out = (long long*)tokens_out_dev; a.tok_out_stride = steps;
    a.past_append = g->past; a.trace = logits_trace_dev; a.B = B;
    int* len_dev = g->pos_dev + 2;
    hipLaunchKernelGGL(k_set_int, dim3(1), dim3(1), 0, st, len_dev, 1);
    a.t_dev = len_dev;

    StepIO io{g->past, pstride, 1, g->logits};
    auto one_step = [&](hipStream_t s, int phase) -> int {
        g->att_nw = wmar_gpt::phase_waves(phase);
        int rc = enqueue_step(g, B, io, s);
        if (rc) return rc;
        g->span_begin(WMAR_T_SAMPLE, s);
        rc = launch_sample_fused(a, s);
        g->span_end(s);
        if (rc) return rc;
        hipLaunchKernelGGL(k_advance3, dim3(1), dim3(1), 0, s, g->pos_dev);
        return launch_status("k_advance3");
    };

    if (g->timing) WMAR_HIP_CHECK(hipEventRecord(g->ev0, st));
    if (sp->use_graph) {
        unsigned long long key[12] = {(unsigned long long)B, (unsigned long long)steps, (unsigned long long)(uintptr_t)q_dev,
                                      (unsigned long long)(uintptr_t)tokens_out_dev, (unsigned long long)(uintptr_t)logits_trace_dev,
                                      wm ? (unsigned long long)(uintptr_t)wm->table_dev : 0ull,
                                      wm ? (unsigned long long)wm->n_rows : 0ull,
                                      wm ? ((unsigned long long)wm->seed_strategy << 40) | ((unsigned long long)wm->context_size << 20) | (unsigned long long)wm->spatial_dim : 0ull,
                                      0ull, 0ull, (unsigned long long)sp->top_k, 0ull};
        float fd = wm ? wm->delta : 0.f, ft = sp->temperature;
        memcpy(&key[8], &fd, 4); memcpy(&key[9], &ft, 4); memcpy(&key[11], &sp->top_p, 8);
        bool need[wmar_gpt::N_PHASE] = {false, false, false};
        for (int n = 0; n < steps; ++n) need[g->att_phase(n + 1, B)] = true;
        int gs = 1;
        {
            static int env_gs = -1;
            if (env_gs < 0) { const char* e = getenv("WMAR_GRAPH_STEPS"); env_gs = e ? atoi(e) : 0; }
            const int want = env_gs > 0 ? env_gs : WMAR_GRAPH_STEPS_DEFAULT;
            const int n_need = (int)need[0] + (int)need[1] + (int)need[2];
            if (n_need == 1 && want > 1 && steps % want == 0) gs = want;
        }
        key[1] |= (unsigned long long)gs << 32;
        if (memcmp(key, g->graph_key, sizeof(key)) != 0) g->gr.drop();
        bool have = true;
        for (int ph = 0; ph < wmar_gpt::N_PHASE; ++ph) have = have && (!need[ph] || g->gr.exec[ph]);
        if (!have) {
            g->gr.drop();
            for (int ph = 0; ph < wmar_gpt::N_PHASE; ++ph) {
                if (!need[ph]) continue;
                const int rc = g->gr.capture(ph, [&](hipStream_t s) {
                    int r = WMAR_OK;
                    for (int k = 0; k < gs && r == WMAR_OK; ++k) r = one_step(s, ph);
                    return r;
                });
                if (rc) return rc;
            }
            memcpy(g->graph_key, key, sizeof(key));
        }
        for (int n = 0; n < steps; n += gs)
            if (int rc = g->gr.replay(g->att_phase(n + 1, B), st)) return rc;
        if (int rc = g->gr.replayed(st)) return rc;
        { StepPlan pl(g, B, io, nullptr); if (!pl.small && pl.proj_xr) g->xr_enqueued = true; if (pl.persist) g->ps_enqueued = true; }
        if (g->timing) WMAR_HIP_CHECK(hipEventSynchronize(g->gr.done));
    } else {
        g->span_on = g->timing != 0;
        int rc = WMAR_OK;
        for (int n = 0; n < steps && rc == WMAR_OK; ++n) rc = one_step(st, g->att_phase(n + 1, B));
        g->span_on = false;
        if (rc) return rc;
        if (g->timing) {
            WMAR_HIP_CHECK(hipEventRecord(g->gr.done, st));
            WMAR_HIP_CHECK(hipStreamSynchronize(st));
            g->span_collect();
        }
    }
    if (g->timing) {
        float ms = 0;
        WMAR_HIP_CHECK(hipEventElapsedTime(&ms, g->ev0, g->gr.done));
        g->step_ms = ms / steps;
    }
    return WMAR_OK;
}

int wmar_gpt_generate(wmar_gpt* g, const wmar_wm_ctx* wm, const wmar_sample_params* sp, const int64_t* cond_dev,
                      int64_t B, int32_t steps, const float* q_dev, int64_t* tokens_out_dev,
                      float* logits_trace_dev, void* stream) {
    WMAR_REQUIRE(g, "generate: null argument");
    return run_with_fallback("generate: the in-launch barrier flag is up on the two-launch path",
                             [&] { return gpt_generate_once(g, wm, sp, cond_dev, B, steps, q_dev, tokens_out_dev, logits_trace_dev, stream); },
                             [&] { return gpt_sync_failed(g, (hipStream_t)stream); });
}

static int gpt_generate_hooked_once(wmar_gpt* g, const wmar_sample_params* sp, const int64_t* cond_dev, int64_t B, int32_t steps,
                                    const float* q_dev, int64_t* tokens_out_dev, const HookIO& hk, void* stream) {
    WMAR_REQUIRE(g && sp && cond_dev && q_dev && tokens_out_dev && hk.logits && hk.past && hk.hook, "generate_hooked: null argument");
    WMAR_REQUIRE(B >= 1 && B <= g->Bmax, "generate_hooked: batch %lld outside 1..%d", (long long)B, g->Bmax);
    WMAR_REQUIRE(steps >= 1 && steps <= g->Tmax, "generate_hooked: steps %d outside 1..block_size %d", steps, g->Tmax);
    WMAR_REQUIRE(hk.past_stride >= (long long)steps + 1, "generate_hooked: past_stride %lld below steps + 1 = %d", hk.past_stride, steps + 1);
    WMAR_REQUIRE(!(sp->top_p >= 0) || sp->top_p <= 1.0, "`top_p` has to be a float > 0 and < 1, but is %f", sp->top_p);
    hipStream_t st = (hipStream_t)stream;
    const long long pstride = hk.past_stride;
    if (int rc = gpt_inject(g, st)) return rc;
    WMAR_HIP_CHECK(hipMemcpy2DAsync(hk.past, pstride * 8, cond_dev, 8, 8, (size_t)B, hipMemcpyDeviceToDevice, st));
    WMAR_HIP_CHECK(hipMemsetAsync(g->pos_dev, 0, 8, st));
    int* len_dev = g->pos_dev + 2;
    hipLaunchKernelGGL(k_set_int, dim3(1), dim3(1), 0, st, len_dev, 1);

    SampArgs a{};
    a.wm = make_wm(nullptr);
    a.logits = hk.logits; a.V = g->V; a.past = hk.past; a.past_stride = pstride; a.t_dev = len_dev;
    a.temperature = sp->temperature; a.top_k = sp->top_k; a.use_top_p = sp->top_p >= 0;
    a.top_p_thr = (float)(1.0 - sp->top_p);
    a.q = q_dev; a.q_step_stride = (long long)B * g->V; a.step_dev = g->step_dev;
    a.scratch = a.V > 65536 ? g->scratch : nullptr;
    a.tok_out = (long long*)tokens_out_dev; a.tok_out_stride = steps;
    a.past_append = hk.past; a.trace = nullptr; a.B = B;

    StepIO io{hk.past, pstride, 1, hk.logits};
    auto step_a = [&](hipStream_t s, int phase) -> int {
        g->att_nw = wmar_gpt::phase_waves(phase);
        return enqueue_step(g, B, io, s);
    };
    auto step_b = [&](hipStream_t s) -> int {
        if (int rc = launch_sample_fused(a, s)) return rc;
        hipLaunchKernelGGL(k_advance3, dim3(1), dim3(1), 0, s, g->pos_dev);
        return launch_status("k_advance3");
    };
    constexpr int SLOT_B = wmar_gpt::N_PHASE;
    if (sp->use_graph) {
        unsigned long long key[12] = {(unsigned long long)B, (unsigned long long)steps, (unsigned long long)(uintptr_t)q_dev,
                                      (unsigned long long)(uintptr_t)tokens_out_dev, (unsigned long long)(uintptr_t)hk.logits,
                                      (unsigned long long)(uintptr_t)hk.past, (unsigned long long)pstride, 0ull, 0ull, 0ull,
                                      (unsigned long long)sp->top_k, 0ull};
        const float ft = sp->temperature;
        memcpy(&key[9], &ft, 4); memcpy(&key[11], &sp->top_p, 8);
        bool need[wmar_gpt::N_PHASE] = {false, false, false};
        for (int n = 0; n < steps; ++n) need[g->att_phase(n + 1, B)] = true;
        if (memcmp(key, g->hook_key, sizeof(key)) != 0) g->grh.drop();
        bool have = g->grh.exec[SLOT_B] != nullptr;
        for (int ph = 0; ph < wmar_gpt::N_PHASE; ++ph) have = have && (!need[ph] || g->grh.exec[ph]);
        if (!have) {
            g->grh.drop();
            memset(g->hook_key, 0, sizeof(g->hook_key));
            for (int ph = 0; ph < wmar_gpt::N_PHASE; ++ph) {
                if (!need[ph]) continue;
                if (int rc = g->grh.capture(ph, [&](hipStream_t s) { return step_a(s, ph); })) return rc;
            }
            if (int rc = g->grh.capture(SLOT_B, step_b)) return rc;
            memcpy(g->hook_key, key, sizeof(key));
        }
    }
    { StepPlan pl(g, B, io, nullptr); if (!pl.small && pl.proj_xr) g->xr_enqueued = true; if (pl.persist) g->ps_enqueued = true; }
    int rc = WMAR_OK;
    for (int n = 0; n < steps && rc == WMAR_OK; ++n) {
        const int ph = g->att_phase(n + 1, B);
        rc = sp->use_graph ? g->grh.replay(ph, st) : step_a(st, ph);
        if (rc == WMAR_OK) rc = call_hook(hk, n, (long long)n + 1);
        if (rc == WMAR_OK) rc = sp->use_graph ? g->grh.replay(SLOT_B, st) : step_b(st);
    }
    if (sp->use_graph) { if (int r = g->grh.replayed(st)) return rc ? rc : r; }
    return rc;
}

int wmar_gpt_generate_hooked(wmar_gpt* g, const wmar_sample_params* sp, const int64_t* cond_dev, int64_t B, int32_t steps,
                             const float* q_dev, int64_t* tokens_out_dev, float* logits_io_dev, int64_t* past_io_dev,
                             int64_t past_stride, wmar_logits_hook hook, void* user, void* stream) {
    WMAR_REQUIRE(g, "generate_hooked: null argument");
    const HookIO hk{logits_io_dev, (long long*)past_io_dev, (long long)past_stride, hook, user};
    return run_with_fallback("generate_hooked: the in-launch barrier flag is up on the two-launch path",
                             [&] { return gpt_generate_hooked_once(g, sp, cond_dev, B, steps, q_dev, tokens_out_dev, hk, stream); },
                             [&] { return gpt_sync_failed(g, (hipStream_t)stream); });
}

}
```

### wmar_amd/csrc/sampler.h

```cpp
#pragma once
#include "common.h"

namespace wmar {

struct WmDev {
    const uint32_t* table;
    long long n_rows;
    long long row_words;
    int seed_mode, h, S;
    float delta;
    int enabled;
};

inline WmDev make_wm(const wmar_wm_ctx* wm) {
    WmDev d{};
    if (wm) {
        d.table = wm->table_dev;
        d.n_rows = wm->n_rows;
        d.row_words = (wm->vocab_size + 31) / 32;
        d.seed_mode = wm->seed_strategy;
        d.h = wm->context_size;
        d.S = wm->spatial_dim;
        d.delta = wm->delta;
        d.enabled = 1;
    }
    return d;
}

struct SampArgs {
    WmDev wm;
    const float* logits;
    long long V;
    const long long* past;
    long long past_stride;
    long long t_host;
    const int* t_dev;
    float temperature;
    int top_k;
    int use_top_p;
    float top_p_thr;
    const float* q;
    long long q_step_stride;
    const int* step_dev;
    float* scratch;
    long long* tok_out;
    long long tok_out_stride;
    long long* past_append;
    float* trace;
    long long B;
    const float* logits_uncond;
    const float* cfg_scale;
    const float* logits_img;
    float g_text, g_image;
    const uint32_t* allow;
    const int* gather;
    long long Vsrc;
};

int launch_sample_fused(const SampArgs& a, hipStream_t st);

struct CfgMixArgs {
    const float* cond;
    const float* img;
    const float* uncond;
    float* out;
    long long V, B;
    const float* scale;
    const int* step_dev;
    float g_text, g_image;
};

int launch_cfg_mix(const CfgMixArgs& a, hipStream_t st);

struct HookIO {
    float* logits;
    long long* past;
    long long past_stride;
    wmar_logits_hook hook;
    void* user;
};

inline int call_hook(const HookIO& h, int step, long long t) {
    const int r = h.hook(h.user, (int32_t)step, (int64_t)t);
    if (r != 0) { set_error("the logits hook returned %d at step %d: generation stopped", r, step); return WMAR_ECALLBACK; }
    return WMAR_OK;
}

struct GumbelArgs {
    const float* logits;
    const float* logits_uncond;
    const float* cfg_scale;
    const int* step_dev;
    const int* t_dev;
    long long V, B;
    const float* log_rs;
    long long key_row_stride;
    int use_sampling;
    float temp, top_p;
    int top_k;
    long long* tok_out;
    long long tok_out_stride;
    long long* past_append;
    long long past_stride;
};

int launch_gumbel_sample(const GumbelArgs& a, hipStream_t st);

struct GumbelCtxArgs {
    const long long* ids;
    long long ids_stride;
// ... 12 lines not shown
```

### wmar_amd/csrc/watermark.hip

```cpp
#include "sampler.h"
#include "../../include/wmar_math.h"

namespace wmar {

__device__ __forceinline__ const uint32_t* wm_row(const WmDev& wm, const long long* past, long long t) {
    if (!wm.enabled) return nullptr;
    long long r = ctx_row(past, t, wm.seed_mode, wm.h, wm.S);
    if (r < 0 || r >= wm.n_rows) return nullptr;
    return wm.table + r * wm.row_words;
}

__global__ __launch_bounds__(256) void k_wm_bias(WmDev wm, float* logits, long long V, const long long* past,
                                                 long long t, long long past_stride) {
    const long long b = blockIdx.y;
    const uint32_t* row = wm_row(wm, past + b * past_stride, t);
    if (!row) return;
    float* lg = logits + b * V;
    const float d = wm.delta;
    for (long long w = blockIdx.x * blockDim.x + threadIdx.x; w * 32 < V; w += (long long)gridDim.x * blockDim.x) {
        uint32_t bits = row[w];
        if (!bits) continue;
        long long v0 = w * 32;
        for (int j = 0; j < 32 && v0 + j < V; ++j)
            if ((bits >> j) & 1u) lg[v0 + j] = lg[v0 + j] + d;
    }
}

__device__ __forceinline__ float cfg_mix2(float c, float u, float scale) {
    const float dlt = c - u;
    const float sc = dlt * scale;
    return u + sc;
}
__device__ __forceinline__ float cfg_mix3(float full, float im, float u, float g_text, float g_image) {
    const float d1 = im - u;
    const float t1 = g_image * d1;
    const float s1 = u + t1;
    const float d2 = full - im;
    const float t2 = g_text * d2;
    return s1 + t2;
}

template <bool VEC>
__global__ __launch_bounds__(256) void k_cfg_mix(CfgMixArgs a) {
    const long long b = blockIdx.y;
    const long long off = b * a.V;
    const bool three = a.img != nullptr;
    const float scale = three ? 0.f : a.scale[a.step_dev ? *a.step_dev : 0];
    const long long stride = (long long)gridDim.x * blockDim.x;
    if (VEC) {
        const long long n4 = a.V >> 2;
        const float4* c4 = reinterpret_cast<const float4*>(a.cond + off);
        const float4* u4 = reinterpret_cast<const float4*>(a.uncond + off);
// ... 54 lines not shown
__device__ __forceinline__ uint32_t block_max_u32(uint32_t v, unsigned long long* red) {
    for (int o = 32; o > 0; o >>= 1) v = max(v, (uint32_t)__shfl_xor((int)v, o));
    const int w = threadIdx.x >> 6, l = threadIdx.x & 63;
    if (l == 0) red[w] = v;
    __syncthreads();
    uint32_t s = 0;
    for (int i = 0; i < SAMP_WAVES; ++i) s = max(s, (uint32_t)red[i]);
    return s;
}

template <bool ASC_MASS>
__device__ __forceinline__ int scan_hist(const unsigned long long* hist, unsigned long long need_or_base, float thr,
                                         unsigned long long* other) {
    const int l = threadIdx.x & 63;
    unsigned long long h0, h1, h2, h3;
    if (ASC_MASS) {
        h0 = hist[4 * l], h1 = hist[4 * l + 1], h2 = hist[4 * l + 2], h3 = hist[4 * l + 3];
    } else {
        h0 = hist[255 - 4 * l], h1 = hist[254 - 4 * l], h2 = hist[253 - 4 * l], h3 = hist[252 - 4 * l];
    }
    unsigned long long tot = h0 + h1 + h2 + h3;
    unsigned long long inc = tot;
    for (int o = 1; o < 64; o <<= 1) {
        unsigned long long n = __shfl_up(inc, o);
        if (l >= o) inc += n;
    }
    unsigned long long exc = inc - tot;
    unsigned long long c0 = exc + h0, c1 = c0 + h1, c2 = c1 + h2, c3 = c2 + h3;
    int hit = -1;
    unsigned long long before = 0;
    if (ASC_MASS) {
        const unsigned long long base = need_or_base;
        if (!(wmar_fx_to_f32(base + c0) <= thr)) { hit = 0; before = exc; }
        else if (!(wmar_fx_to_f32(base + c1) <= thr)) { hit = 1; before = c0; }
        else if (!(wmar_fx_to_f32(base + c2) <= thr)) { hit = 2; before = c1; }
        else if (!(wmar_fx_to_f32(base + c3) <= thr)) { hit = 3; before = c2; }
    } else {
        const unsigned long long need = need_or_base;
        if (c0 >= need) { hit = 0; before = exc; }
        else if (c1 >= need) { hit = 1; before = c0; }
        else if (c2 >= need) { hit = 2; before = c1; }
        else if (c3 >= need) { hit = 3; before = c2; }
    }
    unsigned long long m = __ballot(hit >= 0);
    if (m == 0) { *other = __shfl(inc, 0); return -1; }
    int first = __ffsll((long long)m) - 1;
    int hit_f = __shfl(hit, first);
    unsigned long long before_f = __shfl(before, first);
    *other = before_f;
    int bucket = 4 * first + hit_f;
    return ASC_MASS ? bucket : 255 - bucket;
}

template <int EPT, bool PLAIN = false>
__global__ __launch_bounds__(SAMP_THREADS) void k_sample_fused(SampArgs a) {
    constexpr int N_HIST = 12, N_RED = 5;
    __shared__ unsigned long long hist_all[N_HIST][256];
    __shared__ unsigned long long red_all[N_RED][SAMP_WAVES];
    __shared__ float red_f[SAMP_WAVES];
    __shared__ int red_i[SAMP_WAVES];
    __shared__ float q_lds[(EPT > 0 && EPT <= 16) ? EPT * SAMP_THREADS : 1];
    __shared__ float surv_x[EPT > 0 ? SAMP_THREADS : 1];
    __shared__ int surv_v[EPT > 0 ? SAMP_THREADS : 1];
    __shared__ int surv_n;
    if (threadIdx.x == 0) surv_n = 0;
    static_assert(sizeof(hist_all) + sizeof(red_all) + sizeof(q_lds) + 2 * SAMP_WAVES * 4 + 2 * SAMP_THREADS * 4 + 4 <= 160 * 1024,
                  "k_sample_fused: static LDS beyond the 160 KB of a gfx950 CU (the noise row alone is 64 KB: gfx950 only)");
    for (int i = threadIdx.x; i < N_HIST * 256; i += SAMP_THREADS) (&hist_all[0][0])[i] = 0;

    const long long b = blockIdx.x;
    const long long V = a.V;
    const int tid = threadIdx.x;
    const long long t = a.t_dev ? (long long)*a.t_dev : a.t_host;
    const long long step = a.step_dev ? (long long)*a.step_dev : 0;
    const long long* past = a.past ? a.past + b * a.past_stride : nullptr;
    const uint32_t* grow = (past || a.wm.seed_mode == WMAR_SEED_FIXED) ? wm_row(a.wm, past, t) : nullptr;
    const int* gth = a.gather;
    const long long Vs = gth ? a.Vsrc : V;
#define WMAR_SRC(v) (gth ? (long long)gth[v] : (long long)(v))
    const float* lg = a.logits + b * Vs;
    const float* ul = a.logits_uncond ? a.logits_uncond + b * Vs : nullptr;
    const float* il = a.logits_img ? a.logits_img + b * Vs : nullptr;
    const float cfg = (ul && !il) ? a.cfg_scale[step] : 0.f;
    const float* q = a.q + step * a.q_step_stride + b * Vs;
    float* x = a.scratch + b * V;
    float* trace = a.trace ? a.trace + (step * a.B + b) * Vs : nullptr;
    const float T = a.temperature;
    const float delta = a.wm.delta;
    float xr[EPT > 0 ? EPT : 1];

#define WMAR_FOR_ROW(BODY)                                                                   \
    if (EPT > 0) {                                                                           \
        _Pragma("unroll") for (int i_ = 0; i_ < (EPT > 0 ? EPT : 1); ++i_) {                \
            const long long v = tid + (long long)i_ * SAMP_THREADS;                          \
            if (v < V) { const float xv = xr[i_]; BODY }                                     \
        }                                                                                    \
    } else {                                                                                 \
        for (long long v = tid; v < V; v += SAMP_THREADS) { const float xv = x[v]; BODY }    \
    }

    uint32_t kmax = 0;
    constexpr int QN = (EPT > 0 && EPT <= 16) ? EPT : 1;
    float qpre[QN];
    if (EPT > 0 && EPT <= 16) {
#pragma unroll
        for (int i = 0; i < QN; ++i) {
            const long long v = tid + (long long)i * SAMP_THREADS;
            if (PLAIN) qpre[i] = __builtin_nontemporal_load(q + (v < V ? v : V - 1));
            else qpre[i] = v < V ? q[WMAR_SRC(v)] : 1.f;
        }
    }
#define WMAR_PARK_Q()                                                                        \
    if (EPT > 0 && EPT <= 16) {                                                              \
        _Pragma("unroll") for (int i = 0; i < QN; ++i) q_lds[tid + i * SAMP_THREADS] = qpre[i]; \
    }
    if (EPT > 0 && PLAIN) {
        constexpr int CH = EPT > 8 ? 8 : (EPT > 0 ? EPT : 1);
        const uint32_t* gp = grow ? grow : reinterpret_cast<const uint32_t*>(lg);
#pragma unroll
        for (int c0 = 0; c0 < (EPT > 0 ? EPT : 1); c0 += CH) {
            float lv[CH];
            uint32_t gw[CH];
#pragma unroll
// ... 26 lines not shown
            for (int j = 0; j < CH; ++j) {
                const int i = c0 + j;
                const long long v = tid + (long long)i * SAMP_THREADS;
                const long long sv = v < V ? WMAR_SRC(v) : 0;
                lv[j] = v < V ? lg[sv] : 0.f;
                if (il && v < V) lv[j] = cfg_mix3(lv[j], il[sv], ul[sv], a.g_text, a.g_image);
                else if (ul && v < V) lv[j] = cfg_mix2(lv[j], ul[sv], cfg);
            }
#pragma unroll
            for (int j = 0; j < CH; ++j) {
                const int i = c0 + j;
                const long long v = tid + (long long)i * SAMP_THREADS;
                if (v < V) {
                    float xv = lv[j];
                    const long long sv = WMAR_SRC(v);
                    if (trace) trace[sv] = xv;
                    if (grow && ((grow[sv >> 5] >> (sv & 31)) & 1u)) xv = xv + delta;
                    if (a.allow && !((a.allow[sv >> 5] >> (sv & 31)) & 1u)) xv = -INFINITY;
                    xv = xv / T;
                    xr[i] = xv;
                    if (a.scratch) x[v] = xv;
                    kmax = max(kmax, wmar_f32_key(xv));
                }
            }
        }
    } else {
        for (long long v = tid; v < V; v += SAMP_THREADS) {
            const long long sv = WMAR_SRC(v);
            float xv = lg[sv];
            if (il) xv = cfg_mix3(xv, il[sv], ul[sv], a.g_text, a.g_image);
            else if (ul) xv = cfg_mix2(xv, ul[sv], cfg);
            if (trace) trace[sv] = xv;
            if (grow && ((grow[sv >> 5] >> (sv & 31)) & 1u)) xv = xv + delta;
            if (a.allow && !((a.allow[sv >> 5] >> (sv & 31)) & 1u)) xv = -INFINITY;
            xv = xv / T;
            x[v] = xv;
            kmax = max(kmax, wmar_f32_key(xv));
        }
    }
    WMAR_PARK_Q()
#undef WMAR_PARK_Q
    kmax = block_max_u32(kmax, red_all[0]);
    const float m = wmar_key_f32(kmax);
    const uint32_t NEG_INF_KEY = 0x00800000u;

    uint32_t thr_key = 0;
    unsigned long long n_alive = ~0ull;
    if (a.top_k > 0 && (long long)a.top_k < V) {
        uint32_t prefix = 0, mask = 0;
        unsigned long long need = (unsigned long long)a.top_k;
        for (int pass = 3; pass >= 0; --pass) {
            unsigned long long* hist = hist_all[3 - pass];
            if (pass == 3) {
#define WMAR_TOPBYTE(V_, XV_)                                                                         \
                {                                                                                         \
                    const bool active = (V_) < V;                                                         \
                    const uint32_t d = active ? (wmar_f32_key(XV_) >> 24) : 0xffffffffu;                  \
                    const unsigned long long act = __ballot(active);                                      \
                    if (act) {                                                                            \
                        const int leader = __ffsll((long long)act) - 1;                                   \
                        const uint32_t dl = (uint32_t)__shfl((int)d, leader);                             \
                        const unsigned long long same = __ballot(d == dl);                                \
                        uint32_t* h32 = reinterpret_cast<uint32_t*>(hist);       \
                        if ((tid & 63) == leader) atomicAdd(&h32[2 * dl], (uint32_t)__popcll(same));      \
                        else if (active && d != dl) atomicAdd(&h32[2 * d], 1u);                           \
                    }                                                                                     \
                }
                if (EPT > 0) {
#pragma unroll
                    for (int i_ = 0; i_ < (EPT > 0 ? EPT : 1); ++i_) {
                        if ((long long)i_ * SAMP_THREADS >= V) break;
                        const long long v = tid + (long long)i_ * SAMP_THREADS;
                        WMAR_TOPBYTE(v, xr[i_])
                    }
                } else {
                    for (long long v0 = 0; v0 < V; v0 += SAMP_THREADS) {
                        const long long v = v0 + tid;
                        const float xv = v < V ? x[v] : 0.f;
                        WMAR_TOPBYTE(v, xv)
                    }
                }
#undef WMAR_TOPBYTE
            } else {
                WMAR_FOR_ROW({
                    const uint32_t k = wmar_f32_key(xv);
                    if ((k & mask) == prefix) atomicAdd(&hist[(k >> (8 * pass)) & 255u], 1ull);
                })
            }
            __syncthreads();
            unsigned long long above;
            const int bkt = scan_hist<false>(hist, need, 0.f, &above);
            prefix |= (uint32_t)bkt << (8 * pass);
            mask |= 0xffu << (8 * pass);
            need -= above;
        }
        thr_key = prefix;
        n_alive = (unsigned long long)a.top_k - need + hist_all[3][prefix & 255u];
    }
    if (thr_key <= NEG_INF_KEY) thr_key = NEG_INF_KEY + 1;

    float best = -INFINITY;
    int besti = 0;
    if (EPT > 0 && n_alive <= (unsigned long long)SAMP_THREADS) {
        WMAR_FOR_ROW({
            if (wmar_f32_key(xv) >= thr_key) { const int s_ = atomicAdd(&surv_n, 1); surv_x[s_] = xv; surv_v[s_] = (int)v; }
        })
        __syncthreads();
        const bool my = tid < surv_n;
        const float cx = my ? surv_x[tid] : 0.f;
        const long long cv = my ? (long long)surv_v[tid] : 0;
        const uint32_t ck = wmar_f32_key(cx);
        const float ce = wmar_expf(cx - m);
        uint32_t bkey = 0;
        long long bidx = 0;
        if (a.use_top_p) {
            const unsigned long long S = block_sum_u64(my ? wmar_fx(ce) : 0ull, red_all[1]);
            const float Sf = wmar_fx_to_f32(S);
            const unsigned long long mass = my ? wmar_fx(ce / Sf) : 0ull;
            const float thr = a.top_p_thr;
            uint32_t prefix = 0, mask = 0;
            unsigned long long base = 0;
            bool all_pass = false;
            for (int pass = 3; pass >= 0; --pass) {
                unsigned long long* hist = hist_all[4 + 3 - pass];
                if (my && (ck & mask) == prefix) atomicAdd(&hist[(ck >> (8 * pass)) & 255u], mass);
                __syncthreads();
                unsigned long long below;
                const int bkt = scan_hist<true>(hist, base, thr, &below);
                if (bkt < 0) { all_pass = true; break; }
                prefix |= (uint32_t)bkt << (8 * pass);
                mask |= 0xffu << (8 * pass);
                base += below;
            }
            if (!all_pass) {
                bkey = prefix;
                const unsigned long long cnt = block_sum_u64((my && ck == bkey) ? 1ull : 0ull, red_all[2]);
                if (cnt > 1) {
                    uint32_t ipre = 0, imask = 0;
                    for (int pass = 3; pass >= 0; --pass) {
                        unsigned long long* hist = hist_all[8 + 3 - pass];
                        if (my && ck == bkey && (((uint32_t)cv) & imask) == ipre)
                            atomicAdd(&hist[(((uint32_t)cv) >> (8 * pass)) & 255u], mass);
                        __syncthreads();
                        unsigned long long below;
                        const int bkt = scan_hist<true>(hist, base, thr, &below);
                        ipre |= (uint32_t)(bkt < 0 ? 255 : bkt) << (8 * pass);
                        imask |= 0xffu << (8 * pass);
                        base += below;
                    }
                    bidx = (long long)ipre;
                }
            } else {
                bkey = kmax;
                bidx = (long long)block_max_u32((my && ck == kmax) ? (uint32_t)cv : 0u, red_all[3]);
            }
        }
        const bool kept = my && (ck > bkey || (ck == bkey && cv >= bidx));
        const unsigned long long S2 = block_sum_u64(kept ? wmar_fx(ce) : 0ull, red_all[4]);
        const float Sf2 = wmar_fx_to_f32(S2);
        if (kept) {
            const float qv = (EPT <= 16) ? q_lds[cv] : q[WMAR_SRC(cv)];
            best = (ce / Sf2) / qv;
            besti = (int)cv;
        }
    } else {

    uint32_t bkey = 0;
    long long bidx = 0;
    if (a.use_top_p) {
        unsigned long long S = 0;
        WMAR_FOR_ROW({
            if (wmar_f32_key(xv) >= thr_key) S += wmar_fx(wmar_expf(xv - m));
        })
        S = block_sum_u64(S, red_all[1]);
        const float Sf = wmar_fx_to_f32(S);
        const float thr = a.top_p_thr;
        uint32_t prefix = 0, mask = 0;
        unsigned long long base = 0;
        bool all_pass = false;
        for (int pass = 3; pass >= 0 && !all_pass; --pass) {
            unsigned long long* hist = hist_all[4 + 3 - pass];
            WMAR_FOR_ROW({
                const uint32_t k = wmar_f32_key(xv);
                if (k >= thr_key && (k & mask) == prefix)
                    atomicAdd(&hist[(k >> (8 * pass)) & 255u], wmar_fx(wmar_expf(xv - m) / Sf));
            })
            __syncthreads();
            unsigned long long below;
            const int bkt = scan_hist<true>(hist, base, thr, &below);
            if (bkt < 0) { all_pass = true; break; }
            prefix |= (uint32_t)bkt << (8 * pass);
            mask |= 0xffu << (8 * pass);
            base += below;
        }
        if (!all_pass) {
            bkey = prefix;
            unsigned long long cnt = 0;
            WMAR_FOR_ROW({ cnt += (wmar_f32_key(xv) == bkey); })
            cnt = block_sum_u64(cnt, red_all[2]);
            if (cnt > 1) {
                uint32_t ipre = 0, imask = 0;
                for (int pass = 3; pass >= 0; --pass) {
                    unsigned long long* hist = hist_all[8 + 3 - pass];
                    WMAR_FOR_ROW({
                        if (wmar_f32_key(xv) == bkey && (((uint32_t)v) & imask) == ipre)
                            atomicAdd(&hist[(((uint32_t)v) >> (8 * pass)) & 255u], wmar_fx(wmar_expf(xv - m) / Sf));
                    })
                    __syncthreads();
                    unsigned long long below;
                    const int bkt = scan_hist<true>(hist, base, thr, &below);
                    ipre |= (uint32_t)(bkt < 0 ? 255 : bkt) << (8 * pass);
                    imask |= 0xffu << (8 * pass);
                    base += below;
                }
                bidx = (long long)ipre;
            }
        } else {
            bkey = kmax;
            uint32_t imax = 0;
            WMAR_FOR_ROW({ if (wmar_f32_key(xv) == kmax) imax = max(imax, (uint32_t)v); })
            bidx = (long long)block_max_u32(imax, red_all[3]);
        }
    }

    unsigned long long S2 = 0;
    WMAR_FOR_ROW({
        const uint32_t k = wmar_f32_key(xv);
        const bool kept = k >= thr_key && (k > bkey || (k == bkey && v >= bidx));
        if (kept) S2 += wmar_fx(wmar_expf(xv - m));
    })
    S2 = block_sum_u64(S2, red_all[4]);
    const float Sf2 = wmar_fx_to_f32(S2);
    if (EPT > 0) {
        constexpr int CH = EPT > 16 ? 16 : (EPT > 0 ? EPT : 1);
#pragma unroll
        for (int c0 = 0; c0 < (EPT > 0 ? EPT : 1); c0 += CH) {
            float qv[CH];
#pragma unroll
            for (int j = 0; j < CH; ++j) {
                const long long v = tid + (long long)(c0 + j) * SAMP_THREADS;
                if (EPT <= 16) qv[j] = q_lds[tid + ((c0 + j) % QN) * SAMP_THREADS];
                else qv[j] = v < V ? q[WMAR_SRC(v)] : 1.f;
            }
#pragma unroll
            for (int j = 0; j < CH; ++j) {
                const int i = c0 + j;
                const long long v = tid + (long long)i * SAMP_THREADS;
                if (v < V) {
                    const float xv = xr[i];
                    const uint32_t k = wmar_f32_key(xv);
                    const bool kept = k >= thr_key && (k > bkey || (k == bkey && v >= bidx));
                    const float e = kept ? wmar_expf(xv - m) : 0.0f;
                    const float r = (e / Sf2) / qv[j];
                    if (r > best) { best = r; besti = (int)v; }
                }
            }
        }
    } else {
        for (long long v = tid; v < V; v += SAMP_THREADS) {
            const float xv = x[v];
            const uint32_t k = wmar_f32_key(xv);
            const bool kept = k >= thr_key && (k > bkey || (k == bkey && v >= bidx));
            const float e = kept ? wmar_expf(xv - m) : 0.0f;
            const float r = (e / Sf2) / q[WMAR_SRC(v)];
            if (r > best) { best = r; besti = (int)v; }
        }
    }
    }
#undef WMAR_FOR_ROW
    for (int o = 32; o > 0; o >>= 1) {
        float ob = __shfl_xor(best, o);
        int oi = __shfl_xor(besti, o);
        if (ob > best || (ob == best && oi < besti)) { best = ob; besti = oi; }
    }
    if ((tid & 63) == 0) { red_f[tid >> 6] = best; red_i[tid >> 6] = besti; }
    __syncthreads();
    if (tid == 0) {
        for (int i = 1; i < SAMP_WAVES; ++i)
            if (red_f[i] > best || (red_f[i] == best && red_i[i] < besti)) { best = red_f[i]; besti = red_i[i]; }
        const long long tokv = WMAR_SRC(besti);
        a.tok_out[b * a.tok_out_stride + step] = tokv;
        if (a.past_append) a.past_append[b * a.past_stride + t] = tokv;
    }
#undef WMAR_SRC
}

struct DetArgs {
    WmDev wm;
    double gamma;
    const long long* codes;
    long long L;
    int* n_scored;
    int* n_green;
    double* pval;
    signed char* mask;
    long long mask_stride;
};

__device__ __forceinline__ long long det_num_ngrams(int seed_mode, int h, long long L, long long S) {
    if (seed_mode != WMAR_SEED_SPATIAL) return L - h;
    if (h == 1) return L - 1;
    return (S - 1) * (S - 1);
}

__device__ __forceinline__ void det_ngram_pos(int seed_mode, int h, long long S, long long i, long long* pos) {
    if (seed_mode != WMAR_SEED_SPATIAL) {
        for (int j = 0; j <= h; ++j) pos[j] = i + j;
    } else if (h == 1) {
        long long cell = i + 1;
        long long r = cell / S, c = cell % S;
        pos[0] = (c == 0) ? (r - 1) * S : cell - 1;
        pos[1] = cell;
    } else {
        long long r = i / (S - 1), c = i % (S - 1);
        pos[0] = r * S + c; pos[1] = r * S + c + 1; pos[2] = (r + 1) * S + c; pos[3] = (r + 1) * S + c + 1;
    }
}

__device__ double betainc_int(long long a, long long bb, double x) {
    if (a <= 0) return __longlong_as_double(0x7ff8000000000000ll);
    long long n = a + bb - 1;
    double lt = lgamma((double)n + 1.0) - lgamma((double)a + 1.0) - lgamma((double)(n - a) + 1.0) +
                (double)a * log(x) + (double)(n - a) * log1p(-x);
    double term = exp(lt), sum = term;
    double odds = x / (1.0 - x);
    for (long long k = a; k < n; ++k) {
        term *= ((double)(n - k) / (double)(k + 1)) * odds;
        sum += term;
    }
    return sum > 1.0 ? 1.0 : sum;
}

__global__ __launch_bounds__(256) void k_detect(DetArgs a) {
    __shared__ int red_s[4], red_g[4];
    const long long b = blockIdx.x;
    const long long* codes = a.codes + b * a.L;
    const int h = a.wm.h, n = h + 1;
// ... 3 lines not shown
    }
    const long long cnt = det_num_ngrams(a.wm.seed_mode, h, a.L, S);
    signed char* mask = a.mask ? a.mask + b * a.mask_stride : nullptr;
    if (mask)
        for (int i = threadIdx.x; i < h; i += blockDim.x) mask[i] = -1;
    int ns = 0, ng = 0;
    const bool spatial = a.wm.seed_mode == WMAR_SEED_SPATIAL;
    for (long long i = threadIdx.x; i < cnt; i += blockDim.x) {
        long long pi[4], pj[4], ti[4];
        bool dup = false;
        long long sum = 0, tgt;
        if (spatial) {
            det_ngram_pos(a.wm.seed_mode, h, S, i, pi);
            for (int k = 0; k < n; ++k) ti[k] = codes[pi[k]];
            for (long long j = 0; j < i && !dup; ++j) {
                det_ngram_pos(a.wm.seed_mode, h, S, j, pj);
                bool same = true;
                for (int k = 0; k < n; ++k) same = same && (codes[pj[k]] == ti[k]);
                dup = same;
            }
            for (int k = 0; k < h; ++k) sum += ti[k];
            tgt = ti[h];
        } else {
            for (long long j = 0; j < i && !dup; ++j) {
                bool same = true;
                for (int k = 0; k < n && same; ++k) same = codes[j + k] == codes[i + k];
                dup = same;
            }
            for (int k = 0; k < h; ++k) sum += codes[i + k];
            tgt = codes[i + h];
        }
        int g = 0;
        if (!dup) {
            long long row = a.wm.seed_mode == WMAR_SEED_FIXED ? 0 : sum;
            if (row >= 0 && row < a.wm.n_rows && tgt >= 0 && tgt < a.wm.row_words * 32)
                g = (a.wm.table[row * a.wm.row_words + (tgt >> 5)] >> (tgt & 31)) & 1u;
            ns += 1;
            ng += g;
        }
        if (mask) mask[h + i] = dup ? -1 : (signed char)g;
    }
    for (int o = 32; o > 0; o >>= 1) { ns += __shfl_xor(ns, o); ng += __shfl_xor(ng, o); }
    if ((threadIdx.x & 63) == 0) { red_s[threadIdx.x >> 6] = ns; red_g[threadIdx.x >> 6] = ng; }
    __syncthreads();
    if (threadIdx.x == 0) {
        ns = red_s[0] + red_s[1] + red_s[2] + red_s[3];
        ng = red_g[0] + red_g[1] + red_g[2] + red_g[3];
        a.n_scored[b] = ns;
        a.n_green[b] = ng;
        a.pval[b] = betainc_int(ng, 1 + (long long)ns - ng, a.gamma);
    }
}

int launch_sample_fused(const SampArgs& a, hipStream_t st) {
    const bool plain = !a.gather && !a.logits_uncond && !a.logits_img && !a.allow && !a.trace;
    if (a.V <= 16ll * SAMP_THREADS && plain) hipLaunchKernelGGL((k_sample_fused<16, true>), dim3((unsigned)a.B), dim3(SAMP_THREADS), 0, st, a);
    else if (a.V <= 16ll * SAMP_THREADS) hipLaunchKernelGGL(k_sample_fused<16>, dim3((unsigned)a.B), dim3(SAMP_THREADS), 0, st, a);
    else if (a.V <= 64ll * SAMP_THREADS) hipLaunchKernelGGL(k_sample_fused<64>, dim3((unsigned)a.B), dim3(SAMP_THREADS), 0, st, a);
    else hipLaunchKernelGGL(k_sample_fused<0>, dim3((unsigned)a.B), dim3(SAMP_THREADS), 0, st, a);
    return launch_status("k_sample_fused");
}

}

using namespace wmar;

static int check_wm(const wmar_wm_ctx* wm, int64_t V) {
    WMAR_REQUIRE(wm->table_dev && wm->n_rows > 0, "watermark table missing");
    WMAR_REQUIRE(wm->vocab_size == V, "watermark vocab %lld != logits vocab %lld", (long long)wm->vocab_size, (long long)V);
    WMAR_REQUIRE(wm->seed_strategy >= 0 && wm->seed_strategy <= 2, "bad seed strategy");
    if (wm->seed_strategy == WMAR_SEED_SPATIAL)
        WMAR_REQUIRE(wm->context_size == 1 || wm->context_size == 3,
                     "Spatial seeding only implemented for context size in [1,3]");
    WMAR_REQUIRE(wm->context_size >= 0 && wm->context_size <= WMAR_MAX_CONTEXT, "context size %d unsupported (0..%d)", wm->context_size,
                 WMAR_MAX_CONTEXT);
    return WMAR_OK;
}

extern "C" {

int wmar_wm_process_logits(const wmar_wm_ctx* wm, float* logits_dev, int64_t B, const int64_t* past_ids_dev,
                           int64_t t, int64_t past_stride, void* stream) {
    WMAR_REQUIRE(wm && logits_dev && (past_ids_dev || t == 0 || wm->seed_strategy == WMAR_SEED_FIXED), "process_logits: null argument");
    WMAR_REQUIRE(t >= 0, "process_logits: negative context length");
    if (int rc = check_wm(wm, wm->vocab_size)) return rc;
    if (B == 0) return WMAR_OK;
    if (!past_ids_dev && wm->seed_strategy != WMAR_SEED_FIXED) return WMAR_OK;
    WmDev d = make_wm(wm);
    long long words = d.row_words;
    dim3 grid((unsigned)((words + 255) / 256), (unsigned)B);
    hipLaunchKernelGGL(k_wm_bias, grid, dim3(256), 0, (hipStream_t)stream, d, logits_dev, (long long)wm->vocab_size,
                       (const long long*)past_ids_dev, (long long)t, (long long)past_stride);
    return launch_status("k_wm_bias");
}

int wmar_sample_fused(const wmar_wm_ctx* wm, const float* logits_dev, int64_t B, int64_t V,
                      const int64_t* past_ids_dev, int64_t t, int64_t past_stride, float temperature,
                      int32_t top_k, double top_p, const float* q_dev, float* scratch_dev,
                      int64_t* tok_out_dev, void* stream) {
    WMAR_REQUIRE(logits_dev && q_dev && scratch_dev && tok_out_dev, "sample_fused: null argument");
    WMAR_REQUIRE(V > 0 && V < (1ll << 31), "sample_fused: bad vocab");
    WMAR_REQUIRE(!(top_p >= 0) || top_p <= 1.0, "`top_p` has to be a float > 0 and < 1, but is %f", top_p);
    if (wm) {
        if (int rc = check_wm(wm, V)) return rc;
        WMAR_REQUIRE(past_ids_dev || t == 0 || wm->seed_strategy == WMAR_SEED_FIXED, "sample_fused: past_ids required");
        if (!past_ids_dev && wm->seed_strategy != WMAR_SEED_FIXED) wm = nullptr;
    }
    if (B == 0) return WMAR_OK;
    SampArgs a{};
    a.wm = make_wm(wm);
    a.logits = logits_dev;
    a.V = V;
    a.past = (const long long*)past_ids_dev;
    a.past_stride = past_stride;
    a.t_host = t;
    a.temperature = temperature;
    a.top_k = top_k;
    a.use_top_p = top_p >= 0;
    a.top_p_thr = (float)(1.0 - top_p);
    a.q = q_dev;
    a.scratch = scratch_dev;
    a.tok_out = (long long*)tok_out_dev;
    a.tok_out_stride = 1;
    a.B = B;
    return launch_sample_fused(a, (hipStream_t)stream);
}

int wmar_cfg_mix(const float* cond_dev, const float* img_dev, const float* uncond_dev, float* out_dev, int64_t B, int64_t V,
                 const float* scale_dev, const int32_t* step_dev, float g_text, float g_image, void* stream) {
    WMAR_REQUIRE(cond_dev && uncond_dev && out_dev, "cfg_mix: null argument");
    WMAR_REQUIRE(img_dev || scale_dev, "cfg_mix: the two-way form needs its scale");
    WMAR_REQUIRE(V > 0 && V < (1ll << 31) && B >= 0 && B <= 65535, "cfg_mix: bad shape");
    if (B == 0) return WMAR_OK;
    CfgMixArgs a{};
    a.cond = cond_dev; a.img = img_dev; a.uncond = uncond_dev; a.out = out_dev; a.V = V; a.B = B;
    a.scale = scale_dev; a.step_dev = step_dev; a.g_text = g_text; a.g_image = g_image;
    return launch_cfg_mix(a, (hipStream_t)stream);
}

int wmar_cham_sample(const wmar_wm_ctx* wm, const float* logits3_dev, int64_t B, int64_t V, const int64_t* past_ids_dev,
                     int64_t t, int64_t past_stride, float temperature, double top_p, float guidance_scale_text,
                     float guidance_scale_image, const uint32_t* allow_dev, const int32_t* allow_ids_dev, int32_t n_allow,
                     const float* q_dev, float* scratch_dev, int64_t* tok_out_dev, void* stream) {
    WMAR_REQUIRE(logits3_dev && q_dev && scratch_dev && tok_out_dev, "cham_sample: null argument");
    WMAR_REQUIRE(V > 0 && V < (1ll << 31), "cham_sample: bad vocab");
    WMAR_REQUIRE(!(top_p >= 0) || top_p <= 1.0, "`top_p` has to be a float > 0 and < 1, but is %f", top_p);
    if (wm) {
        if (int rc = check_wm(wm, V)) return rc;
        WMAR_REQUIRE(past_ids_dev || wm->seed_strategy == WMAR_SEED_FIXED, "cham_sample: past_ids required");
    }
    if (B == 0) return WMAR_OK;
    SampArgs a{};
    a.wm = make_wm(wm);
    a.logits = logits3_dev;
    a.logits_img = logits3_dev + B * V;
    a.logits_uncond = logits3_dev + 2 * B * V;
    a.g_text = guidance_scale_text;
    a.g_image = guidance_scale_image;
    a.allow = allow_dev;
    a.V = V;
    if (allow_ids_dev && n_allow > 0) { a.gather = allow_ids_dev; a.Vsrc = V; a.V = n_allow; }
    a.past = (const long long*)past_ids_dev;
    a.past_stride = past_stride;
    a.t_host = t;
    a.temperature = temperature;
    a.top_k = 0;
    a.use_top_p = top_p >= 0;
    a.top_p_thr = (float)(1.0 - top_p);
    a.q = q_dev;
    a.scratch = scratch_dev;
    a.tok_out = (long long*)tok_out_dev;
    a.tok_out_stride = 1;
    a.B = B;
    return launch_sample_fused(a, (hipStream_t)stream);
}

int64_t wmar_detect_num_ngrams(int32_t seed_strategy, int32_t context_size, int64_t L) {
    if (seed_strategy != WMAR_SEED_SPATIAL) return L - context_size;
// ... 38 lines not shown
```

### wmar_amd/models/engine.py

```python
from __future__ import annotations

import ctypes as C
from typing import Dict, Optional

import numpy as np
import torch

from .. import _lib
from ..utils.synth import GPTConfig, VQConfig


def _require_cuda(t: torch.Tensor, what: str):
    if not t.is_cuda:
        raise RuntimeError(f"wmar_amd: {what} must live on the MI355X (no CPU implementation)")


class _Engine:

    _prefix = ""

    def _create(self, config, state: Dict[str, torch.Tensor], keep, device, max_batch: int, dtype=torch.float32):
        self.device = torch.device(device)
        self.max_batch = int(max_batch)
        self._L = _lib.load()
# ... 102 lines not shown
                                                    _lib.stream_ptr(self.device)))
        return logits

    def generate(self, cond: torch.Tensor, steps: int, q: torch.Tensor, temperature=1.0, top_k=None, top_p=None,
                 wm_ctx: Optional[_lib.WmCtx] = None, use_graph: bool = True, trace_logits: bool = False):
        _require_cuda(cond, "conditioning")
        _require_cuda(q, "q")
        cond = cond.to(torch.int64).contiguous().view(-1)
        B = cond.shape[0]
        V = self.cfg.vocab_size
        assert q.shape == (steps, B, V) and q.dtype == torch.float32 and q.is_contiguous()
        out = torch.empty(B, steps, dtype=torch.int64, device=self.device)
        trace = torch.empty(steps, B, V, dtype=torch.float32, device=self.device) if trace_logits else None
        sp = _lib.SampleParams(float(temperature), int(top_k) if top_k else 0,
                               float(top_p) if top_p is not None else -1.0, 1 if use_graph else 0)
        with torch.cuda.device(self.device):
            _lib.check(self._L.wmar_gpt_generate(
                self._h, C.byref(wm_ctx) if wm_ctx is not None else None, C.byref(sp), cond.data_ptr(), B, int(steps),
                q.data_ptr(), out.data_ptr(), trace.data_ptr() if trace is not None else None,
                _lib.stream_ptr(self.device)))
            _lib.check(self._L.wmar_gpt_check(self._h, _lib.stream_ptr(self.device)))
        return (out, trace) if trace_logits else out

    def generate_hooked(self, cond: torch.Tensor, steps: int, q: torch.Tensor, processor, temperature=1.0, top_k=None, top_p=None,
                        use_graph: bool = True) -> torch.Tensor:
        _require_cuda(cond, "conditioning")
        _require_cuda(q, "q")
        cond = cond.to(torch.int64).contiguous().view(-1)
        B = cond.shape[0]
        V = self.cfg.vocab_size
        assert q.shape == (steps, B, V) and q.dtype == torch.float32 and q.is_contiguous()
        out = torch.empty(B, steps, dtype=torch.int64, device=self.device)
        sp = _lib.SampleParams(float(temperature), int(top_k) if top_k else 0,
                               float(top_p) if top_p is not None else -1.0, 1 if use_graph else 0)
        with torch.cuda.device(self.device):
            hook = _LogitsHook(processor, B, V, steps + 1, self.device, positional=False)
            hook.finish(self._L.wmar_gpt_generate_hooked(
                self._h, C.byref(sp), cond.data_ptr(), B, int(steps), q.data_ptr(), out.data_ptr(), hook.logits.data_ptr(),
                hook.past.data_ptr(), hook.past.stride(0), hook.cfunc, None, _lib.stream_ptr(self.device)))
            _lib.check(self._L.wmar_gpt_check(self._h, _lib.stream_ptr(self.device)))
        return out

    def profile_role(self, role: str, B: int, kv_len: int = 128, iters: int = 96) -> float:
        out = C.c_double()
        with torch.cuda.device(self.device):
            _lib.check(self._L.wmar_gpt_profile_role(self._h, self.T_CLASSES.index(role), B, kv_len, iters,
                                                     _lib.stream_ptr(self.device), C.byref(out)))
        return out.value

    def plan_info(self, B: int) -> Dict[str, str]:
        buf = C.create_string_buffer(2048)
        _lib.check(self._L.wmar_gpt_plan_info(self._h, int(B), buf, len(buf)))
        return dict(kv.split("=", 1) for kv in buf.value.decode().split(";"))

    def set_attention_phases(self, one_wave_upto: int, two_waves_upto: int):
        _lib.check(self._L.wmar_gpt_set_attention_phases(self._h, int(one_wave_upto), int(two_waves_upto)))

    def set_timing(self, on: bool):
        self._L.wmar_gpt_set_timing(self._h, 1 if on else 0)

    T_CLASSES = ["embed", "qkv", "attn", "proj", "resid", "fc1", "fc2", "head", "sample"]

    def get_timing(self):
        n = len(self.T_CLASSES)
        us = (C.c_double * n)()
        calls = (C.c_int64 * n)()
        step = C.c_double()
        self._L.wmar_gpt_get_timing(self._h, us, calls, C.byref(step))
        return {k: (us[i], calls[i]) for i, k in enumerate(self.T_CLASSES)}, step.value


class VQGANEngine(_TokenizerEngine):

    _prefix = "wmar_vq"

    def __init__(self, cfg: VQConfig, state: Dict[str, torch.Tensor], max_batch: int = 64, device="cuda"):
        self.cfg = cfg
        self._out_channels, self._code_dim = cfg.out_ch, cfg.embed_dim
        c = _lib.VqConfig()
        c.ch, c.num_res_blocks, c.resolution = cfg.ch, cfg.num_res_blocks, cfg.resolution
        c.in_channels, c.out_ch, c.z_channels = cfg.in_channels, cfg.out_ch, cfg.z_channels
        c.embed_dim, c.n_embed, c.n_levels = cfg.embed_dim, cfg.n_embed, len(cfg.ch_mult)
        for i, m in enumerate(cfg.ch_mult):
            c.ch_mult[i] = m
        c.n_attn_res = len(cfg.attn_resolutions)
        for i, r in enumerate(cfg.attn_resolutions):
            c.attn_resolutions[i] = r
        c.max_batch = int(max_batch)
        self._create(c, state, lambda k: not k.startswith("loss."), device, max_batch)


class RAREngine(_Engine):

    _prefix = "wmar_rar"

    def __init__(self, cfg, state: Dict[str, torch.Tensor], max_batch: int = 64, device="cuda"):
        self.cfg = cfg
        c = _lib.RarConfig(cfg.hidden_size, cfg.num_hidden_layers, cfg.num_attention_heads, cfg.intermediate_size,
                           cfg.image_seq_len, cfg.codebook_size, cfg.condition_num_classes, int(max_batch))
        self._create(c, state, lambda k: k != "attn_mask", device, max_batch)

    def _staging(self, class_ids: torch.Tensor, cfg_scales: Optional[torch.Tensor]):
        _require_cuda(class_ids, "class ids")
        class_ids = class_ids.to(torch.int64).contiguous().view(-1)
        out = torch.empty(class_ids.shape[0], self.cfg.image_seq_len, dtype=torch.int64, device=self.device)
        if cfg_scales is None:
# ... 175 lines not shown
```

Baseline: 58.74 images/s.

## Split top-k sampling across workgroups, fold embedding into layer-0 QKV, ticket-advance counters

Top-k sampling is now split into two launches. A select kernel runs four workgroups per row and collects candidates, and a finish kernel picks the winner from them. If a row overflows the candidate cap, the finish kernel falls back to the fused per-row sampler. The token and position embedding gather is folded into the layer-0 QKV kernel, which removes a separate embed launch. In captured loops, the counter advance kernel is replaced by an atomic ticket at the end of the finish kernel. These changes aim to raise parallelism in the sampling step and cut per-step launch overhead in the decode loop, at the cost of an extra workspace and more complex control paths.

```diff
diff --git a/include/wmar_hip.h b/include/wmar_hip.h
--- a/include/wmar_hip.h
+++ b/include/wmar_hip.h
@@ -60,6 +60,7 @@
                       const int64_t* past_ids_dev, int64_t t, int64_t past_stride, float temperature,
                       int32_t top_k, double top_p, const float* q_dev, float* scratch_dev,
                       int64_t* tok_out_dev, void* stream);
+int wmar_sample_split_info(int32_t* cap_out, int32_t* used_out, int32_t* fellback_host, int64_t n_rows);
 
 int wmar_detect(const wmar_wm_ctx* wm, double gamma, const int64_t* codes_dev, int64_t B, int64_t L,
                 int32_t* n_scored_dev, int32_t* n_green_dev, double* pval_dev, int8_t* mask_dev,
@@ -91,6 +92,8 @@
 int wmar_gpt_generate(wmar_gpt* g, const wmar_wm_ctx* wm, const wmar_sample_params* sp, const int64_t* cond_dev,
                       int64_t B, int32_t steps, const float* q_dev, int64_t* tokens_out_dev,
                       float* logits_trace_dev, void* stream);
+
+int wmar_gpt_counters(wmar_gpt* g, int32_t* out4_host, void* stream);
 
 typedef int (*wmar_logits_hook)(void* user, int32_t step, int64_t t);
 
diff --git a/wmar_amd/_lib.py b/wmar_amd/_lib.py
--- a/wmar_amd/_lib.py
+++ b/wmar_amd/_lib.py
@@ -8,9 +8,9 @@
 
 SYMBOLS = [
     "wmar_last_error", "wmar_version", "wmar_key_row_words", "wmar_key_table_rows", "wmar_key_table_build",
-    "wmar_key_greenlist", "wmar_wm_process_logits", "wmar_sample_fused", "wmar_detect", "wmar_detect_num_ngrams",
+    "wmar_key_greenlist", "wmar_wm_process_logits", "wmar_sample_fused", "wmar_sample_split_info", "wmar_detect", "wmar_detect_num_ngrams",
     "wmar_gpt_create", "wmar_gpt_destroy", "wmar_gpt_device_bytes", "wmar_gpt_decode_step", "wmar_gpt_generate",
-    "wmar_gpt_set_timing", "wmar_gpt_set_attention_phases", "wmar_gpt_get_timing", "wmar_gpt_profile_role", "wmar_gpt_plan_info", "wmar_gpt_check", "wmar_rar_create", "wmar_rar_destroy",
+    "wmar_gpt_counters", "wmar_gpt_set_timing", "wmar_gpt_set_attention_phases", "wmar_gpt_get_timing", "wmar_gpt_profile_role", "wmar_gpt_plan_info", "wmar_gpt_check", "wmar_rar_create", "wmar_rar_destroy",
     "wmar_rar_device_bytes", "wmar_rar_forward_position", "wmar_rar_generate", "wmar_vq_create", "wmar_vq_destroy", "wmar_vq_device_bytes",
     "wmar_vq_decode", "wmar_vq_encode", "wmar_vq_probe_conv", "wmar_vq_probe_attn", "wmar_vq_probe_argmin", "wmar_mvq_create", "wmar_mvq_destroy", "wmar_mvq_device_bytes", "wmar_mvq_decode",
     "wmar_mvq_encode", "wmar_gumbel_key_build", "wmar_gumbel_sample", "wmar_gumbel_score", "wmar_gumbel_key_rows", "wmar_gumbel_score_ctx", "wmar_rar_generate_gumbel", "wmar_rar_generate_gumbel_ctx", "wmar_rar_check", "wmar_rar_launch_status",
@@ -117,6 +117,7 @@
     L.wmar_key_greenlist.argtypes = [C.POINTER(KeyParams), C.c_uint64, vp]
     L.wmar_wm_process_logits.argtypes = [C.POINTER(WmCtx), vp, i64, vp, i64, i64, vp]
     L.wmar_sample_fused.argtypes = [C.POINTER(WmCtx), vp, i64, i64, vp, i64, i64, f32, i32, f64, vp, vp, vp, vp]
+    L.wmar_sample_split_info.argtypes = [C.POINTER(i32), C.POINTER(i32), vp, i64]
     L.wmar_detect.argtypes = [C.POINTER(WmCtx), f64, vp, i64, i64, vp, vp, vp, vp, i64, vp]
     L.wmar_detect_num_ngrams.restype = i64
     L.wmar_detect_num_ngrams.argtypes = [i32, i32, i64]
@@ -149,6 +150,7 @@
     L.wmar_gpt_decode_step.argtypes = [vp, vp, i64, i32, vp, vp]
     L.wmar_gpt_generate.argtypes = [vp, C.POINTER(WmCtx), C.POINTER(SampleParams), vp, i64, i32, vp, vp, vp, vp]
     L.wmar_gpt_set_timing.argtypes = [vp, i32]
+    L.wmar_gpt_counters.argtypes = [vp, C.POINTER(i32), vp]
     L.wmar_gpt_set_attention_phases.argtypes = [vp, i32, i32]
     L.wmar_gpt_profile_role.argtypes = [vp, i32, i64, i32, i32, vp, C.POINTER(f64)]
     L.wmar_gpt_get_timing.argtypes = [vp, C.POINTER(f64), C.POINTER(i64), C.POINTER(f64)]
diff --git a/wmar_amd/csrc/decoder_kernels.h b/wmar_amd/csrc/decoder_kernels.h
--- a/wmar_amd/csrc/decoder_kernels.h
+++ b/wmar_amd/csrc/decoder_kernels.h
@@ -725,6 +725,13 @@
     int nkeep;
     unsigned long long* trace;
     unsigned long long* trace_chunks;
+    const float* tok_emb;
+    const float* pos_emb;
+    const long long* tok;
+    long long tok_stride;
+    int tok_use_pos;
+    const int* pos_dev;
+    int B, K;
 };
 
 template <int MTW, int S_IN>
@@ -960,8 +967,9 @@
 }
 
 constexpr int QX_TR_STRIDE = 36;
-template <int S_IN>
+template <int S_IN, bool EMBED = false>
 __global__ __launch_bounds__(512) void k_qkvx_bx(QkvxArgs a) {
+    static_assert(!EMBED || S_IN == 0, "the embedding has nothing to fold");
     constexpr int MTW = 2;
     __shared__ __attribute__((aligned(16))) u32x4 xq[2][2][MTW][3][64];
     __shared__ __attribute__((aligned(16))) float tr_s[4][32 * QX_TR_STRIDE];
@@ -987,12 +995,31 @@
         float4 xvA[MTW], bbA, slA[S_IN > 0 ? S_IN : 1][MTW];
         float4 xvB[MTW], bbB, slB[S_IN > 0 ? S_IN : 1][MTW];
         int skbA = 0, skbB = 0;
+        const float* erow[MTW];
+        const float* prow = nullptr;
+#pragma unroll
+        for (int i = 0; i < MTW; ++i) erow[i] = nullptr;
+        if (EMBED) {
+            const int pos = *a.pos_dev;
+#pragma unroll
+            for (int i = 0; i < MTW; ++i) {
+                const int m = i * 32 + (lane & 31);
+                const long long tk = (m < a.B) ? a.tok[(long long)m * a.tok_stride + (a.tok_use_pos ? pos : 0)] : 0;
+                erow[i] = a.tok_emb + tk * a.K;
+            }
+            prow = a.pos_emb + (long long)pos * a.K;
+        }
 #define WMAR_QX_ISSUE(XV, BB, SL, SKB, C)                                                              \
     {                                                                                                   \
         SKB = kb0 + (C) * QX_CK + sw;                                                                   \
         const int kk = SKB < kb1 ? SKB : kb1 - 1;                                                       \
         const long long idx = (long long)kk * MTW * 64 + lane;                                          \
-        _Pragma("unroll") for (int i = 0; i < MTW; ++i) XV[i] = a.x_in[idx + i * 64];                   \
+        if (EMBED) {                                                                                    \
+            _Pragma("unroll") for (int i = 0; i < MTW; ++i) XV[i] = *(const float4*)(erow[i] + kk * 8 + 4 * half); \
+            BB = *(const float4*)(prow + kk * 8 + 4 * half);                                            \
+        } else {                                                                                        \
+            _Pragma("unroll") for (int i = 0; i < MTW; ++i) XV[i] = a.x_in[idx + i * 64];               \
+        }                                                                                               \
         if (S_IN > 0) {                                                                                 \
             BB = *(const float4*)(a.bias + kk * 8 + 4 * half);                                          \
             _Pragma("unroll") for (int si = 0; si < S_IN; ++si)                                         \
@@ -1005,6 +1032,7 @@
         const bool short_tile = a.n_hi > 0 && (SKB >> 2) >= a.n_hi;                                     \
         _Pragma("unroll") for (int i = 0; i < MTW; ++i) {                                               \
             float4 r = XV[i];                                                                           \
+            if (EMBED) r = make_float4(r.x + BB.x, r.y + BB.y, r.z + BB.z, r.w + BB.w);                 \
             if (S_IN > 0) {                                                                             \
                 float4 t = SL[0][i];                                                                    \
                 _Pragma("unroll") for (int si = 1; si < S_IN; ++si)                                     \
@@ -1160,8 +1188,13 @@
     if (keeper) __syncthreads();
 }
 
-static int launch_qkvx_bx(const QkvxArgs& q, int S_in, hipStream_t st) {
+static int launch_qkvx_bx(const QkvxArgs& q, int S_in, hipStream_t st, bool embed = false) {
     const dim3 grid((unsigned)(8 * q.cap));
+    if (embed) {
+        if (S_in != 0) { set_error("qkvx_bx: the embedding variant folds no slabs (%d)", S_in); return WMAR_EINVAL; }
+        hipLaunchKernelGGL((k_qkvx_bx<0, true>), grid, dim3(512), 0, st, q);
+        return launch_status("k_qkvx_bx<embed>");
+    }
     switch (S_in) {
 #define WMAR_QX_CASE(N) case N: hipLaunchKernelGGL((k_qkvx_bx<N>), grid, dim3(512), 0, st, q); break;
         WMAR_QX_CASE(0) WMAR_QX_CASE(1) WMAR_QX_CASE(2) WMAR_QX_CASE(3) WMAR_QX_CASE(4)
diff --git a/wmar_amd/csrc/gpt.hip b/wmar_amd/csrc/gpt.hip
--- a/wmar_amd/csrc/gpt.hip
+++ b/wmar_amd/csrc/gpt.hip
@@ -47,6 +47,7 @@
     double* stats_q = nullptr;
     float *kcache = nullptr, *vcache = nullptr;
     float *logits = nullptr, *scratch = nullptr;
+    unsigned long long* samp_split = nullptr;
     long long* past = nullptr;
     int *pos_dev = nullptr, *step_dev = nullptr;
     hipEvent_t ev0 = nullptr;
@@ -198,6 +199,7 @@
     bool qkv_bx() const { return S_qx > 0 && MT == 2 && g->layers[0].wqkvx_bx && !g->no_bx && !g->no_bx_qkv; }
     bool fc1_x() const { return MT == 2 && g->layers[0].wfc1x16 && nch_ln2 <= 16; }
     int qx_nkeep() const { const int G = 3 * D / 128; return G >= 4 && S_qx * 4 <= STAT_CHUNKS_MAX ? 4 : 1; }
+    bool embed_in_qkv() const { return qkv_bx() && !getenv("WMAR_EMBED_LAUNCH"); }
     static bool head_narrow() { static int v = -1; if (v < 0) v = getenv("WMAR_HEAD_NARROW") ? 1 : 0; return v != 0; }
     int split_for(int NT, int KB) const { return pick_split(MT % 2 == 0 ? NT * (MT / 2) : NT * MT, KB, 4); }
     GemmArgs base() const {
@@ -248,7 +250,12 @@
         q.trace = g->stamp_slot(l, 0);
         g->span_begin(WMAR_T_QKV, st);
         int rc;
-        if (qkv_bx()) { q.Wp = w.wqkvx_bx; rc = launch_qkvx_bx(q, S_in, st); }
+        const bool emb = !prev_bias && l == 0 && embed_in_qkv();
+        if (emb) {
+            q.x_in = nullptr; q.tok_emb = g->tok_emb; q.pos_emb = g->pos_emb; q.tok = io.tok; q.tok_stride = io.tok_stride;
+            q.tok_use_pos = io.tok_use_pos; q.pos_dev = g->pos_dev; q.B = (int)B; q.K = D;
+        }
+        if (qkv_bx()) { q.Wp = w.wqkvx_bx; rc = launch_qkvx_bx(q, S_in, st, emb); }
         else rc = launch_qkvx(q, MT, S_in, st);
         g->span_end(st);
         xcur = xout;
@@ -466,7 +473,7 @@
         g->ps_enqueued = true;
         return rc;
     }
-    if ((rc = p.embed())) return rc;
+    if (!p.embed_in_qkv() && (rc = p.embed())) return rc;
     if (p.small) {
         for (int l = 0; l < g->L; ++l) {
             if ((rc = p.qkv_small(l))) return rc;
@@ -668,6 +675,7 @@
     WMAR_TRY(g->mem.alloc_zero(&g->vcache, kv, st));
     WMAR_TRY(g->mem.alloc(&g->logits, (size_t)g->Bmax * V));
     WMAR_TRY(g->mem.alloc(&g->scratch, (size_t)g->Bmax * V));
+    if (g->Bmax >= SAMP_SPLIT_MIN_ROWS) WMAR_TRY(g->mem.alloc(&g->samp_split, (sample_split_bytes(g->Bmax) + 7) / 8));
     WMAR_TRY(g->mem.alloc_zero(&g->past, (size_t)g->Bmax * (g->Tmax + 1), st));
     WMAR_TRY(g->mem.alloc(&g->pos_dev, 4));
     WMAR_TRY(g->mem.alloc_zero(&g->xsync, 8 * 64 + 64, st));
@@ -827,9 +835,9 @@
         WMAR_REQUIRE(n > 0 && n < buf_len, "plan_info: buffer of %lld bytes too small", (long long)buf_len);
         return WMAR_OK;
     }
-    char qkv[96], proj[160], fc1[96], fc2[96];
+    char qkv[128], proj[160], fc1[96], fc2[96];
     const int S_in = p.S_fc2 + (p.fc2_hi > 0 ? 1 : 0);
-    if (p.qkv_bx()) snprintf(qkv, sizeof qkv, "k_qkvx_bx<%d> (bf16 pipe, %d K slices)", S_in, p.S_qx);
+    if (p.qkv_bx()) snprintf(qkv, sizeof qkv, "k_qkvx_bx<%d> (bf16 pipe, %d K slices%s)", S_in, p.S_qx, p.embed_in_qkv() ? ", layer 0 gathers the embedding" : "");
     else if (p.S_qx > 0) snprintf(qkv, sizeof qkv, "k_qkvx<%d,%d> (fp32 MFMA, %d K slices)", p.MT, S_in, p.S_qx);
     else snprintf(qkv, sizeof qkv, "k_gemm<EPI_PACKED> (fp32 MFMA, %d K slices) after k_resid_stats", p.S_qkv);
     if (p.proj_xr) snprintf(proj, sizeof proj, "k_bx_xr<%d,4> (bf16 pipe, 4 K slices + XCD-local reduction: residual fold and LN2 statistics inside)", BX_PER);
@@ -843,8 +851,14 @@
               w2 = wmar_gpt::phase_waves(g->att_phase(g->Tmax, B));
     if (w0 == w1 && w1 == w2) snprintf(attn, sizeof attn, "k_attn_decode<%d,%d>", g->hd, w1);
     else snprintf(attn, sizeof attn, "k_attn_decode<%d,%d> (%d / %d / %d waves at 1 / %d / %d cached rows)", g->hd, w1, w0, w1, w2, g->Tmax / 2, g->Tmax);
-    const int n = snprintf(buf, (size_t)buf_len, "qkv=%s;attn=%s;proj=%s;resid=k_resid_stats;resid_launches_per_step=%d;fc1=%s;fc2=%s;head=k_gemm<EPI_LOGITS,LN> (fp32 MFMA);barrier_fallbacks=%d",
-                           qkv, attn, proj, p.proj_xr ? 1 : g->L + 1, fc1, fc2, g->fallbacks);
+    SampArgs sa{};
+    sa.split = g->samp_split; sa.B = B; sa.V = g->V; sa.top_k = 250;
+    const bool split = sample_split_eligible(sa);
+    const int n = snprintf(buf, (size_t)buf_len, "qkv=%s;attn=%s;proj=%s;resid=k_resid_stats;resid_launches_per_step=%d;fc1=%s;fc2=%s;head=k_gemm<EPI_LOGITS,LN> (fp32 MFMA);barrier_fallbacks=%d;"
+                           "sample=%s;advance=%s",
+                           qkv, attn, proj, p.proj_xr ? 1 : g->L + 1, fc1, fc2, g->fallbacks,
+                           split ? "k_sample_select (4 workgroups per row) + k_sample_finish at 0 < top_k <= 1024, k_sample_fused otherwise" : "k_sample_fused",
+                           split && !getenv("WMAR_ADVANCE_LAUNCH") ? "ticket in k_sample_finish (captured loop), k_advance3 (eager, hooked)" : "k_advance3");
     WMAR_REQUIRE(n > 0 && n < buf_len, "plan_info: buffer of %lld bytes too small", (long long)buf_len);
     return WMAR_OK;
 }
@@ -890,6 +904,13 @@
 }
 #endif
 
+
+int wmar_gpt_counters(wmar_gpt* g, int32_t* out4_host, void* stream) {
+    WMAR_REQUIRE(g && out4_host, "counters: null argument");
+    WMAR_HIP_CHECK(hipStreamSynchronize((hipStream_t)stream));
+    WMAR_HIP_CHECK(hipMemcpy(out4_host, g->pos_dev, 16, hipMemcpyDeviceToHost));
+    return WMAR_OK;
+}
 
 int wmar_gpt_set_attention_phases(wmar_gpt* g, int32_t one_wave_upto, int32_t two_waves_upto) {
     WMAR_REQUIRE(g, "set_attention_phases: null argument");
@@ -947,9 +968,13 @@
     a.scratch = a.V > 65536 ? g->scratch : nullptr;
     a.tok_out = (long long*)tokens_out_dev; a.tok_out_stride = steps;
     a.past_append = g->past; a.trace = logits_trace_dev; a.B = B;
+    a.split = g->samp_split;
     int* len_dev = g->pos_dev + 2;
     hipLaunchKernelGGL(k_set_int, dim3(1), dim3(1), 0, st, len_dev, 1);
     a.t_dev = len_dev;
+    const bool ticket = sp->use_graph && sample_split_eligible(a) && !getenv("WMAR_ADVANCE_LAUNCH");
+    hipLaunchKernelGGL(k_set_int, dim3(1), dim3(1), 0, st, g->pos_dev + 3, 0);
+    if (ticket) { a.advance = g->pos_dev; a.ticket = g->pos_dev + 3; }
 
     StepIO io{g->past, pstride, 1, g->logits};
     auto one_step = [&](hipStream_t s, int phase) -> int {
@@ -959,7 +984,7 @@
         g->span_begin(WMAR_T_SAMPLE, s);
         rc = launch_sample_fused(a, s);
         g->span_end(s);
-        if (rc) return rc;
+        if (rc || ticket) return rc;
         hipLaunchKernelGGL(k_advance3, dim3(1), dim3(1), 0, s, g->pos_dev);
         return launch_status("k_advance3");
     };
@@ -971,7 +996,9 @@
                                       wm ? (unsigned long long)(uintptr_t)wm->table_dev : 0ull,
                                       wm ? (unsigned long long)wm->n_rows : 0ull,
                                       wm ? ((unsigned long long)wm->seed_strategy << 40) | ((unsigned long long)wm->context_size << 20) | (unsigned long long)wm->spatial_dim : 0ull,
-                                      0ull, 0ull, (unsigned long long)sp->top_k, 0ull};
+                                      0ull, 0ull, (unsigned long long)(unsigned)sp->top_k, 0ull};
+        key[10] |= (unsigned long long)sample_split_eligible(a) << 32 | (unsigned long long)ticket << 33 |
+                   (unsigned long long)StepPlan(g, B, io, nullptr).embed_in_qkv() << 34;
         float fd = wm ? wm->delta : 0.f, ft = sp->temperature;
         memcpy(&key[8], &fd, 4); memcpy(&key[9], &ft, 4); memcpy(&key[11], &sp->top_p, 8);
         bool need[wmar_gpt::N_PHASE] = {false, false, false};
@@ -1059,6 +1086,7 @@
     a.scratch = a.V > 65536 ? g->scratch : nullptr;
     a.tok_out = (long long*)tokens_out_dev; a.tok_out_stride = steps;
     a.past_append = hk.past; a.trace = nullptr; a.B = B;
+    a.split = g->samp_split;
 
     StepIO io{hk.past, pstride, 1, hk.logits};
     auto step_a = [&](hipStream_t s, int phase) -> int {
@@ -1075,7 +1103,8 @@
         unsigned long long key[12] = {(unsigned long long)B, (unsigned long long)steps, (unsigned long long)(uintptr_t)q_dev,
                                       (unsigned long long)(uintptr_t)tokens_out_dev, (unsigned long long)(uintptr_t)hk.logits,
                                       (unsigned long long)(uintptr_t)hk.past, (unsigned long long)pstride, 0ull, 0ull, 0ull,
-                                      (unsigned long long)sp->top_k, 0ull};
+                                      (unsigned long long)(unsigned)sp->top_k | (unsigned long long)sample_split_eligible(a) << 32 |
+                                          (unsigned long long)StepPlan(g, B, io, nullptr).embed_in_qkv() << 33, 0ull};
         const float ft = sp->temperature;
         memcpy(&key[9], &ft, 4); memcpy(&key[11], &sp->top_p, 8);
         bool need[wmar_gpt::N_PHASE] = {false, false, false};
diff --git a/wmar_amd/csrc/sampler.h b/wmar_amd/csrc/sampler.h
--- a/wmar_amd/csrc/sampler.h
+++ b/wmar_amd/csrc/sampler.h
@@ -55,7 +55,15 @@
     const uint32_t* allow;
     const int* gather;
     long long Vsrc;
+    void* split;
+    int* advance;
+    int* ticket;
 };
+
+constexpr int SAMP_SPLIT_CAP = 1024;
+constexpr int SAMP_SPLIT_MIN_ROWS = 33;
+inline size_t sample_split_bytes(long long B) { return (size_t)B * (4 * SAMP_SPLIT_CAP * 8 + 4 * 4 + 4); }
+bool sample_split_eligible(const SampArgs& a);
 
 int launch_sample_fused(const SampArgs& a, hipStream_t st);
 
diff --git a/wmar_amd/csrc/watermark.hip b/wmar_amd/csrc/watermark.hip
--- a/wmar_amd/csrc/watermark.hip
+++ b/wmar_amd/csrc/watermark.hip
@@ -1,3 +1,6 @@
+#include <mutex>
+#include <vector>
+
 #include "sampler.h"
 #include "../../include/wmar_math.h"
 
@@ -158,8 +161,100 @@
     return ASC_MASS ? bucket : 255 - bucket;
 }
 
-template <int EPT, bool PLAIN = false>
-__global__ __launch_bounds__(SAMP_THREADS) void k_sample_fused(SampArgs a) {
+template <class QLoad>
+__device__ __forceinline__ void sample_compact_tail(const SampArgs& a, unsigned long long (*hist8)[256],
+                                                    unsigned long long (*red4)[SAMP_WAVES], bool my, float cx, long long cv, float m,
+                                                    uint32_t kmax, QLoad qload, float& best, int& besti) {
+    const uint32_t ck = wmar_f32_key(cx);
+    const float ce = wmar_expf(cx - m);
+    uint32_t bkey = 0;
+    long long bidx = 0;
+    if (a.use_top_p) {
+        const unsigned long long S = block_sum_u64(my ? wmar_fx(ce) : 0ull, red4[0]);
+        const float Sf = wmar_fx_to_f32(S);
+        const unsigned long long mass = my ? wmar_fx(ce / Sf) : 0ull;
+        const float thr = a.top_p_thr;
+        uint32_t prefix = 0, mask = 0;
+        unsigned long long base = 0;
+        bool all_pass = false;
+        for (int pass = 3; pass >= 0; --pass) {
+            unsigned long long* hist = hist8[3 - pass];
+            if (my && (ck & mask) == prefix) atomicAdd(&hist[(ck >> (8 * pass)) & 255u], mass);
+            __syncthreads();
+            unsigned long long below;
+            const int bkt = scan_hist<true>(hist, base, thr, &below);
+            if (bkt < 0) { all_pass = true; break; }
+            prefix |= (uint32_t)bkt << (8 * pass);
+            mask |= 0xffu << (8 * pass);
+            base += below;
+        }
+        if (!all_pass) {
+            bkey = prefix;
+            const unsigned long long cnt = block_sum_u64((my && ck == bkey) ? 1ull : 0ull, red4[1]);
+            if (cnt > 1) {
+                uint32_t ipre = 0, imask = 0;
+                for (int pass = 3; pass >= 0; --pass) {
+                    unsigned long long* hist = hist8[4 + 3 - pass];
+                    if (my && ck == bkey && (((uint32_t)cv) & imask) == ipre)
+                        atomicAdd(&hist[(((uint32_t)cv) >> (8 * pass)) & 255u], mass);
+                    __syncthreads();
+                    unsigned long long below;
+                    const int bkt = scan_hist<true>(hist, base, thr, &below);
+                    ipre |= (uint32_t)(bkt < 0 ? 255 : bkt) << (8 * pass);
+                    imask |= 0xffu << (8 * pass);
+                    base += below;
+                }
+                bidx = (long long)ipre;
+            }
+        } else {
+            bkey = kmax;
+            bidx = (long long)block_max_u32((my && ck == kmax) ? (uint32_t)cv : 0u, red4[2]);
+        }
+    }
+    const bool kept = my && (ck > bkey || (ck == bkey && cv >= bidx));
+    const unsigned long long S2 = block_sum_u64(kept ? wmar_fx(ce) : 0ull, red4[3]);
+    const float Sf2 = wmar_fx_to_f32(S2);
+    if (kept) {
+        const float qv = qload(cv);
+        best = (ce / Sf2) / qv;
+        besti = (int)cv;
+    }
+}
+
+__device__ __forceinline__ void sample_write_winner(const SampArgs& a, long long b, long long t, long long step, float best, int besti,
+                                                    float* red_f, int* red_i) {
+    const int tid = threadIdx.x;
+    for (int o = 32; o > 0; o >>= 1) {
+        float ob = __shfl_xor(best, o);
+        int oi = __shfl_xor(besti, o);
+        if (ob > best || (ob == best && oi < besti)) { best = ob; besti = oi; }
+    }
+    if ((tid & 63) == 0) { red_f[tid >> 6] = best; red_i[tid >> 6] = besti; }
+    __syncthreads();
+    if (tid == 0) {
+        for (int i = 1; i < SAMP_WAVES; ++i)
+            if (red_f[i] > best || (red_f[i] == best && red_i[i] < besti)) { best = red_f[i]; besti = red_i[i]; }
+        const long long tokv = a.gather ? (long long)a.gather[besti] : (long long)besti;
+        a.tok_out[b * a.tok_out_stride + step] = tokv;
+        if (a.past_append) a.past_append[b * a.past_stride + t] = tokv;
+    }
+}
+
+__device__ __forceinline__ void topbyte_count(unsigned long long* hist, bool active, uint32_t key) {
+    const uint32_t d = active ? (key >> 24) : 0xffffffffu;
+    const unsigned long long act = __ballot(active);
+    if (act) {
+        const int leader = __ffsll((long long)act) - 1;
+        const uint32_t dl = (uint32_t)__shfl((int)d, leader);
+        const unsigned long long same = __ballot(d == dl);
+        uint32_t* h32 = reinterpret_cast<uint32_t*>(hist);
+        if ((int)(threadIdx.x & 63) == leader) atomicAdd(&h32[2 * dl], (uint32_t)__popcll(same));
+        else if (active && d != dl) atomicAdd(&h32[2 * d], 1u);
+    }
+}
+
+template <int EPT, bool PLAIN>
+__device__ __forceinline__ void sample_fused_row(const SampArgs& a, const long long b) {
     constexpr int N_HIST = 12, N_RED = 5;
     __shared__ unsigned long long hist_all[N_HIST][256];
     __shared__ unsigned long long red_all[N_RED][SAMP_WAVES];
@@ -174,7 +269,6 @@
                   "k_sample_fused: static LDS beyond the 160 KB of a gfx950 CU (the noise row alone is 64 KB: gfx950 only)");
     for (int i = threadIdx.x; i < N_HIST * 256; i += SAMP_THREADS) (&hist_all[0][0])[i] = 0;
 
-    const long long b = blockIdx.x;
     const long long V = a.V;
     const int tid = threadIdx.x;
     const long long t = a.t_dev ? (long long)*a.t_dev : a.t_host;
@@ -307,35 +401,20 @@
         for (int pass = 3; pass >= 0; --pass) {
             unsigned long long* hist = hist_all[3 - pass];
             if (pass == 3) {
-#define WMAR_TOPBYTE(V_, XV_)                                                                         \
-                {                                                                                         \
-                    const bool active = (V_) < V;                                                         \
-                    const uint32_t d = active ? (wmar_f32_key(XV_) >> 24) : 0xffffffffu;                  \
-                    const unsigned long long act = __ballot(active);                                      \
-                    if (act) {                                                                            \
-                        const int leader = __ffsll((long long)act) - 1;                                   \
-                        const uint32_t dl = (uint32_t)__shfl((int)d, leader);                             \
-                        const unsigned long long same = __ballot(d == dl);                                \
-                        uint32_t* h32 = reinterpret_cast<uint32_t*>(hist);       \
-                        if ((tid & 63) == leader) atomicAdd(&h32[2 * dl], (uint32_t)__popcll(same));      \
-                        else if (active && d != dl) atomicAdd(&h32[2 * d], 1u);                           \
-                    }                                                                                     \
-                }
                 if (EPT > 0) {
 #pragma unroll
                     for (int i_ = 0; i_ < (EPT > 0 ? EPT : 1); ++i_) {
                         if ((long long)i_ * SAMP_THREADS >= V) break;
                         const long long v = tid + (long long)i_ * SAMP_THREADS;
-                        WMAR_TOPBYTE(v, xr[i_])
+                        topbyte_count(hist, v < V, wmar_f32_key(xr[i_]));
                     }
                 } else {
                     for (long long v0 = 0; v0 < V; v0 += SAMP_THREADS) {
                         const long long v = v0 + tid;
                         const float xv = v < V ? x[v] : 0.f;
-                        WMAR_TOPBYTE(v, xv)
+                        topbyte_count(hist, v < V, wmar_f32_key(xv));
                     }
                 }
-#undef WMAR_TOPBYTE
             } else {
                 WMAR_FOR_ROW({
                     const uint32_t k = wmar_f32_key(xv);
@@ -364,60 +443,8 @@
         const bool my = tid < surv_n;
         const float cx = my ? surv_x[tid] : 0.f;
         const long long cv = my ? (long long)surv_v[tid] : 0;
-        const uint32_t ck = wmar_f32_key(cx);
-        const float ce = wmar_expf(cx - m);
-        uint32_t bkey = 0;
-        long long bidx = 0;
-        if (a.use_top_p) {
-            const unsigned long long S = block_sum_u64(my ? wmar_fx(ce) : 0ull, red_all[1]);
-            const float Sf = wmar_fx_to_f32(S);
-            const unsigned long long mass = my ? wmar_fx(ce / Sf) : 0ull;
-            const float thr = a.top_p_thr;
-            uint32_t prefix = 0, mask = 0;
-            unsigned long long base = 0;
-            bool all_pass = false;
-            for (int pass = 3; pass >= 0; --pass) {
-                unsigned long long* hist = hist_all[4 + 3 - pass];
-                if (my && (ck & mask) == prefix) atomicAdd(&hist[(ck >> (8 * pass)) & 255u], mass);
-                __syncthreads();
-                unsigned long long below;
-                const int bkt = scan_hist<true>(hist, base, thr, &below);
-                if (bkt < 0) { all_pass = true; break; }
-                prefix |= (uint32_t)bkt << (8 * pass);
-                mask |= 0xffu << (8 * pass);
-                base += below;
-            }
-            if (!all_pass) {
-                bkey = prefix;
-                const unsigned long long cnt = block_sum_u64((my && ck == bkey) ? 1ull : 0ull, red_all[2]);
-                if (cnt > 1) {
-                    uint32_t ipre = 0, imask = 0;
-                    for (int pass = 3; pass >= 0; --pass) {
-                        unsigned long long* hist = hist_all[8 + 3 - pass];
-                        if (my && ck == bkey && (((uint32_t)cv) & imask) == ipre)
-                            atomicAdd(&hist[(((uint32_t)cv) >> (8 * pass)) & 255u], mass);
-                        __syncthreads();
-                        unsigned long long below;
-                        const int bkt = scan_hist<true>(hist, base, thr, &below);
-                        ipre |= (uint32_t)(bkt < 0 ? 255 : bkt) << (8 * pass);
-                        imask |= 0xffu << (8 * pass);
-                        base += below;
-                    }
-                    bidx = (long long)ipre;
-                }
-            } else {
-                bkey = kmax;
-                bidx = (long long)block_max_u32((my && ck == kmax) ? (uint32_t)cv : 0u, red_all[3]);
-            }
-        }
-        const bool kept = my && (ck > bkey || (ck == bkey && cv >= bidx));
-        const unsigned long long S2 = block_sum_u64(kept ? wmar_fx(ce) : 0ull, red_all[4]);
-        const float Sf2 = wmar_fx_to_f32(S2);
-        if (kept) {
-            const float qv = (EPT <= 16) ? q_lds[cv] : q[WMAR_SRC(cv)];
-            best = (ce / Sf2) / qv;
-            besti = (int)cv;
-        }
+        sample_compact_tail(a, hist_all + 4, red_all + 1, my, cx, cv, m, kmax,
+                            [&](long long v_) { return (EPT <= 16) ? q_lds[v_] : q[WMAR_SRC(v_)]; }, best, besti);
     } else {
 
     uint32_t bkey = 0;
@@ -523,21 +550,227 @@
     }
     }
 #undef WMAR_FOR_ROW
-    for (int o = 32; o > 0; o >>= 1) {
-        float ob = __shfl_xor(best, o);
-        int oi = __shfl_xor(besti, o);
-        if (ob > best || (ob == best && oi < besti)) { best = ob; besti = oi; }
-    }
-    if ((tid & 63) == 0) { red_f[tid >> 6] = best; red_i[tid >> 6] = besti; }
+#undef WMAR_SRC
+    sample_write_winner(a, b, t, step, best, besti, red_f, red_i);
+}
+
+template <int EPT, bool PLAIN = false>
+__global__ __launch_bounds__(SAMP_THREADS) void k_sample_fused(SampArgs a) { sample_fused_row<EPT, PLAIN>(a, blockIdx.x); }
+
+struct SplitBufs {
+    unsigned long long* cand;
+    int* cnt;
+    int* fell;
+};
+__host__ __device__ __forceinline__ SplitBufs split_bufs(const SampArgs& a) {
+    SplitBufs s;
+    s.cand = static_cast<unsigned long long*>(a.split);
+    s.cnt = reinterpret_cast<int*>(s.cand + a.B * 4 * SAMP_SPLIT_CAP);
+    s.fell = s.cnt + a.B * 4;
+    return s;
+}
+
+template <int EPT>
+__global__ __launch_bounds__(SAMP_THREADS) void k_sample_select(SampArgs a) {
+    __shared__ unsigned long long hist_all[4][256];
+    __shared__ int wcnt[EPT * SAMP_WAVES];
+    for (int i = threadIdx.x; i < 4 * 256; i += SAMP_THREADS) (&hist_all[0][0])[i] = 0;
+    const int tid = threadIdx.x, w = tid >> 6, l = tid & 63;
+    const long long b = blockIdx.x >> 2;
+    const int j = blockIdx.x & 3;
+    const long long V = a.V;
+    const long long Q = (V + 3) / 4;
+    const long long v0 = j * Q;
+    const long long n = (v0 + Q <= V ? v0 + Q : V) - v0;
+    const SplitBufs sb = split_bufs(a);
+    if (n <= 0) {
+        if (tid == 0) sb.cnt[b * 4 + j] = 0;
+        return;
+    }
+    const long long t = a.t_dev ? (long long)*a.t_dev : a.t_host;
+    const long long step = a.step_dev ? (long long)*a.step_dev : 0;
+    const long long* past = a.past ? a.past + b * a.past_stride : nullptr;
+    const uint32_t* grow = (past || a.wm.seed_mode == WMAR_SEED_FIXED) ? wm_row(a.wm, past, t) : nullptr;
+    const float* lg = a.logits + b * V;
+    float* x = a.scratch ? a.scratch + b * V : nullptr;
+    float* trace = a.trace ? a.trace + (step * a.B + b) * V : nullptr;
+    const float T = a.temperature;
+    const float delta = a.wm.delta;
+    const uint32_t* gp = grow ? grow : reinterpret_cast<const uint32_t*>(lg);
+
+    uint32_t key[EPT];
+    float xr[EPT];
+    constexpr int CH = EPT > 8 ? 8 : EPT;
+#pragma unroll
+    for (int c0 = 0; c0 < EPT; c0 += CH) {
+        float lv[CH];
+        uint32_t gw[CH];
+#pragma unroll
+        for (int k = 0; k < CH; ++k) {
+            const long long o = tid + (long long)(c0 + k) * SAMP_THREADS;
+            const long long vv = v0 + (o < n ? o : n - 1);
+            lv[k] = __builtin_nontemporal_load(lg + vv);
+            gw[k] = gp[vv >> 5];
+        }
+#pragma unroll
+        for (int k = 0; k < CH; ++k) {
+            const long long o = tid + (long long)(c0 + k) * SAMP_THREADS;
+            const long long v = v0 + o;
+            float xv = lv[k];
+            if (o < n) {
+                if (trace) trace[v] = xv;
+                if (grow && ((gw[k] >> (v & 31)) & 1u)) xv = xv + delta;
+                if (T != 1.0f) xv = xv / T;
+                if (x) x[v] = xv;
+            }
+            xr[c0 + k] = xv;
+            key[c0 + k] = wmar_f32_key(xv);
+        }
+    }
     __syncthreads();
-    if (tid == 0) {
-        for (int i = 1; i < SAMP_WAVES; ++i)
-            if (red_f[i] > best || (red_f[i] == best && red_i[i] < besti)) { best = red_f[i]; besti = red_i[i]; }
-        const long long tokv = WMAR_SRC(besti);
-        a.tok_out[b * a.tok_out_stride + step] = tokv;
-        if (a.past_append) a.past_append[b * a.past_stride + t] = tokv;
-    }
-#undef WMAR_SRC
+
+    const uint32_t NEG_INF_KEY = 0x00800000u;
+    uint32_t prefix = 0, mask = 0;
+    unsigned long long need = (unsigned long long)((long long)a.top_k < n ? (long long)a.top_k : n);
+    for (int pass = 3; pass >= 0; --pass) {
+        unsigned long long* hist = hist_all[3 - pass];
+#pragma unroll
+        for (int i = 0; i < EPT; ++i) {
+            if ((long long)i * SAMP_THREADS >= n) break;
+            const bool active = tid + (long long)i * SAMP_THREADS < n;
+            if (pass == 3) topbyte_count(hist, active, key[i]);
+            else if (active && (key[i] & mask) == prefix) atomicAdd(&hist[(key[i] >> (8 * pass)) & 255u], 1ull);
+        }
+        __syncthreads();
+        unsigned long long above;
+        const int bkt = scan_hist<false>(hist, need, 0.f, &above);
+        prefix |= (uint32_t)bkt << (8 * pass);
+        mask |= 0xffu << (8 * pass);
+        need -= above;
+    }
+    const uint32_t thr_key = prefix <= NEG_INF_KEY ? NEG_INF_KEY + 1 : prefix;
+
+    unsigned long long bal[EPT];
+#pragma unroll
+    for (int i = 0; i < EPT; ++i) {
+        const bool c = tid + (long long)i * SAMP_THREADS < n && key[i] >= thr_key;
+        bal[i] = __ballot(c);
+        if (l == 0) wcnt[i * SAMP_WAVES + w] = __popcll(bal[i]);
+    }
+    __syncthreads();
+    constexpr int NPL = EPT * SAMP_WAVES / 64;
+    int h[NPL], tot = 0;
+#pragma unroll
+    for (int k = 0; k < NPL; ++k) { h[k] = wcnt[l * NPL + k]; tot += h[k]; }
+    int inc = tot;
+    for (int o = 1; o < 64; o <<= 1) {
+        const int up = __shfl_up(inc, o);
+        if (l >= o) inc += up;
+    }
+    const int total = __shfl(inc, 63);
+    if (tid == 0) sb.cnt[b * 4 + j] = total;
+    if (total > SAMP_SPLIT_CAP) return;
+    unsigned long long* out = sb.cand + (b * 4 + j) * SAMP_SPLIT_CAP;
+    const int sub = w % NPL;
+    int pre = inc - tot;
+#pragma unroll
+    for (int k = 0; k < NPL; ++k) if (k < sub) pre += h[k];
+#pragma unroll
+    for (int i = 0; i < EPT; ++i) {
+        const int base = __shfl(pre, (i * SAMP_WAVES + w) / NPL);
+        if ((bal[i] >> l) & 1ull) {
+            const int pos = base + __popcll(bal[i] & ((1ull << l) - 1ull));
+            out[pos] = ((unsigned long long)__float_as_uint(xr[i]) << 32) | (unsigned long long)(uint32_t)(v0 + tid + (long long)i * SAMP_THREADS);
+        }
+    }
+}
+
+template <int EPT, bool PLAIN>
+__global__ __launch_bounds__(SAMP_THREADS) void k_sample_finish(SampArgs a) {
+    constexpr int N_HIST = 12, N_RED = 5;
+    __shared__ unsigned long long hist_all[N_HIST][256];
+    __shared__ unsigned long long red_all[N_RED][SAMP_WAVES];
+    __shared__ float red_f[SAMP_WAVES];
+    __shared__ int red_i[SAMP_WAVES];
+    __shared__ float surv_x[SAMP_THREADS];
+    __shared__ int surv_v[SAMP_THREADS];
+    __shared__ int surv_n;
+    const int tid = threadIdx.x;
+    const long long b = blockIdx.x;
+    const SplitBufs sb = split_bufs(a);
+    const long long t = a.t_dev ? (long long)*a.t_dev : a.t_host;
+    const long long step = a.step_dev ? (long long)*a.step_dev : 0;
+    int c[4];
+#pragma unroll
+    for (int j = 0; j < 4; ++j) c[j] = sb.cnt[b * 4 + j];
+    bool fast = c[0] <= SAMP_SPLIT_CAP && c[1] <= SAMP_SPLIT_CAP && c[2] <= SAMP_SPLIT_CAP && c[3] <= SAMP_SPLIT_CAP;
+    if (fast) {
+        if (tid == 0) surv_n = 0;
+        for (int i = tid; i < N_HIST * 256; i += SAMP_THREADS) (&hist_all[0][0])[i] = 0;
+        float cx[4];
+        uint32_t ck[4], ci[4];
+        bool has[4];
+        uint32_t kmax = 0;
+#pragma unroll
+        for (int j = 0; j < 4; ++j) {
+            has[j] = tid < c[j];
+            const unsigned long long e = sb.cand[(b * 4 + j) * SAMP_SPLIT_CAP + (has[j] ? tid : 0)];
+            cx[j] = __uint_as_float((uint32_t)(e >> 32));
+            ci[j] = (uint32_t)e;
+            ck[j] = wmar_f32_key(cx[j]);
+            if (has[j]) kmax = max(kmax, ck[j]);
+        }
+        kmax = block_max_u32(kmax, red_all[0]);
+        const float m = wmar_key_f32(kmax);
+        const unsigned long long total = (unsigned long long)c[0] + c[1] + c[2] + c[3];
+        uint32_t thr_key = 0;
+        unsigned long long n_alive = total;
+        if (total > (unsigned long long)a.top_k) {
+            uint32_t prefix = 0, mask = 0;
+            unsigned long long need = (unsigned long long)a.top_k;
+            for (int pass = 3; pass >= 0; --pass) {
+                unsigned long long* hist = hist_all[3 - pass];
+#pragma unroll
+                for (int j = 0; j < 4; ++j) {
+                    if (pass == 3) topbyte_count(hist, has[j], ck[j]);
+                    else if (has[j] && (ck[j] & mask) == prefix) atomicAdd(&hist[(ck[j] >> (8 * pass)) & 255u], 1ull);
+                }
+                __syncthreads();
+                unsigned long long above;
+                const int bkt = scan_hist<false>(hist, need, 0.f, &above);
+                prefix |= (uint32_t)bkt << (8 * pass);
+                mask |= 0xffu << (8 * pass);
+                need -= above;
+            }
+            thr_key = prefix;
+            n_alive = (unsigned long long)a.top_k - need + hist_all[3][prefix & 255u];
+        }
+        fast = n_alive <= (unsigned long long)SAMP_THREADS;
+        if (fast) {
+#pragma unroll
+            for (int j = 0; j < 4; ++j)
+                if (has[j] && ck[j] >= thr_key) { const int s_ = atomicAdd(&surv_n, 1); surv_x[s_] = cx[j]; surv_v[s_] = (int)ci[j]; }
+            __syncthreads();
+            const bool my = tid < surv_n;
+            const float sx = my ? surv_x[tid] : 0.f;
+            const long long sv = my ? (long long)surv_v[tid] : 0;
+            const float* q = a.q + step * a.q_step_stride + b * a.V;
+            float best = -INFINITY;
+            int besti = 0;
+            sample_compact_tail(a, hist_all + 4, red_all + 1, my, sx, sv, m, kmax,
+                                [&](long long v_) { return __builtin_nontemporal_load(q + v_); }, best, besti);
+            sample_write_winner(a, b, t, step, best, besti, red_f, red_i);
+        }
+    }
+    if (tid == 0) sb.fell[b] = fast ? 0 : 1;
+    if (!fast) sample_fused_row<EPT, PLAIN>(a, b);
+    if (tid == 0 && a.advance) {
+        __threadfence();
+        if (atomicAdd(a.ticket, 1) == (int)a.B - 1) {
+            a.advance[0] += 1; a.advance[1] += 1; a.advance[2] += 1;
+            *a.ticket = 0;
+        }
+    }
 }
 
 struct DetArgs {
@@ -647,8 +880,31 @@
     }
 }
 
+static bool sample_split_off() { const char* e = getenv("WMAR_SAMPLE_FUSED"); return e && *e && *e != '0'; }
+
+static bool sample_split_shape_ok(const SampArgs& a) {
+    return a.B >= SAMP_SPLIT_MIN_ROWS && a.V <= 64ll * SAMP_THREADS && a.top_k > 0 && a.top_k <= SAMP_SPLIT_CAP &&
+           (long long)a.top_k < a.V && !a.gather && !a.allow && !a.logits_uncond && !a.logits_img && !sample_split_off();
+}
+
+bool sample_split_eligible(const SampArgs& a) {
+    return a.split && (reinterpret_cast<uintptr_t>(a.split) & 7u) == 0 && sample_split_shape_ok(a);
+}
+
 int launch_sample_fused(const SampArgs& a, hipStream_t st) {
     const bool plain = !a.gather && !a.logits_uncond && !a.logits_img && !a.allow && !a.trace;
+    const bool split = sample_split_eligible(a);
+    WMAR_REQUIRE(split || !a.advance, "sample: the counter ticket needs the two-launch sampler");
+    if (split) {
+        const dim3 gs((unsigned)(4 * a.B)), gf((unsigned)a.B), blk(SAMP_THREADS);
+        if (a.V <= 16ll * SAMP_THREADS) hipLaunchKernelGGL(k_sample_select<4>, gs, blk, 0, st, a);
+        else hipLaunchKernelGGL(k_sample_select<16>, gs, blk, 0, st, a);
+        if (int rc = launch_status("k_sample_select")) return rc;
+        if (a.V <= 16ll * SAMP_THREADS && plain) hipLaunchKernelGGL((k_sample_finish<16, true>), gf, blk, 0, st, a);
+        else if (a.V <= 16ll * SAMP_THREADS) hipLaunchKernelGGL((k_sample_finish<16, false>), gf, blk, 0, st, a);
+        else hipLaunchKernelGGL((k_sample_finish<64, false>), gf, blk, 0, st, a);
+        return launch_status("k_sample_finish");
+    }
     if (a.V <= 16ll * SAMP_THREADS && plain) hipLaunchKernelGGL((k_sample_fused<16, true>), dim3((unsigned)a.B), dim3(SAMP_THREADS), 0, st, a);
     else if (a.V <= 16ll * SAMP_THREADS) hipLaunchKernelGGL(k_sample_fused<16>, dim3((unsigned)a.B), dim3(SAMP_THREADS), 0, st, a);
     else if (a.V <= 64ll * SAMP_THREADS) hipLaunchKernelGGL(k_sample_fused<64>, dim3((unsigned)a.B), dim3(SAMP_THREADS), 0, st, a);
@@ -659,6 +915,29 @@
 }
 
 using namespace wmar;
+
+namespace {
+struct SplitWs { int dev = -1; hipStream_t st = nullptr; void* buf = nullptr; long long rows = 0; };
+std::mutex g_split_mu;
+std::vector<SplitWs> g_split_ws;
+SplitWs g_split_last;
+
+const SplitWs* split_workspace(long long B, hipStream_t st) {
+    int dev = 0;
+    if (hipGetDevice(&dev) != hipSuccess) return nullptr;
+    SplitWs* p = nullptr;
+    for (SplitWs& w : g_split_ws) if (w.dev == dev && w.st == st) p = &w;
+    if (p && p->rows >= B) return p;
+    hipStreamCaptureStatus cs = hipStreamCaptureStatusNone;
+    if (hipStreamIsCapturing(st, &cs) != hipSuccess || cs != hipStreamCaptureStatusNone) return nullptr;
+    void* nb = nullptr;
+    if (hipMalloc(&nb, sample_split_bytes(B)) != hipSuccess) { (void)hipGetLastError(); return nullptr; }
+    if (!p) { g_split_ws.push_back(SplitWs{}); p = &g_split_ws.back(); p->dev = dev; p->st = st; }
+    else (void)hipFree(p->buf);
+    p->buf = nb; p->rows = B;
+    return p;
+}
+}
 
 static int check_wm(const wmar_wm_ctx* wm, int64_t V) {
     WMAR_REQUIRE(wm->table_dev && wm->n_rows > 0, "watermark table missing");
@@ -718,7 +997,29 @@
     a.tok_out = (long long*)tok_out_dev;
     a.tok_out_stride = 1;
     a.B = B;
+    {
+        std::lock_guard<std::mutex> lk(g_split_mu);
+        g_split_last = SplitWs{};
+        if (sample_split_shape_ok(a)) {
+            if (const SplitWs* ws = split_workspace(B, (hipStream_t)stream)) { a.split = ws->buf; g_split_last = *ws; g_split_last.rows = B; }
+        }
+    }
     return launch_sample_fused(a, (hipStream_t)stream);
+}
+
+int wmar_sample_split_info(int32_t* cap_out, int32_t* used_out, int32_t* fellback_host, int64_t n_rows) {
+    if (cap_out) *cap_out = SAMP_SPLIT_CAP;
+    SplitWs last;
+    { std::lock_guard<std::mutex> lk(g_split_mu); last = g_split_last; }
+    if (used_out) *used_out = last.buf ? 1 : 0;
+    if (fellback_host && last.buf) {
+        WMAR_REQUIRE(n_rows == last.rows, "sample_split_info: %lld rows asked, the last call had %lld", (long long)n_rows, last.rows);
+        SampArgs a{};
+        a.split = last.buf; a.B = last.rows;
+        WMAR_HIP_CHECK(hipDeviceSynchronize());
+        WMAR_HIP_CHECK(hipMemcpy(fellback_host, split_bufs(a).fell, (size_t)last.rows * 4, hipMemcpyDeviceToHost));
+    }
+    return WMAR_OK;
 }
 
 int wmar_cfg_mix(const float* cond_dev, const float* img_dev, const float* uncond_dev, float* out_dev, int64_t B, int64_t V,
diff --git a/wmar_amd/models/engine.py b/wmar_amd/models/engine.py
--- a/wmar_amd/models/engine.py
+++ b/wmar_amd/models/engine.py
@@ -178,6 +178,12 @@
         buf = C.create_string_buffer(2048)
         _lib.check(self._L.wmar_gpt_plan_info(self._h, int(B), buf, len(buf)))
         return dict(kv.split("=", 1) for kv in buf.value.decode().split(";"))
+
+    def counters(self):
+        out = (C.c_int32 * 4)()
+        with torch.cuda.device(self.device):
+            _lib.check(self._L.wmar_gpt_counters(self._h, out, _lib.stream_ptr(self.device)))
+        return tuple(out)
 
     def set_attention_phases(self, one_wave_upto: int, two_waves_upto: int):
         _lib.check(self._L.wmar_gpt_set_attention_phases(self._h, int(one_wave_upto), int(two_waves_upto)))
```

After: 58.43 images/s. No clear change (-0.5%).
